# maropu/spark-data-repair-plugin

Measured on AMD Instinct MI355X. Metric: repaired cells/sec, higher is better.
Workload: dtype f32 gradients (LightGBM's score_t), exact int64 fixed-point histogram sums, f64 scores

## Files before the change

### spark-data-repair-plugin_amd/csrc/rgbm.hip

```cpp
#include <hip/hip_runtime.h>
#include <algorithm>
#include <atomic>
#include <condition_variable>
#include <chrono>
#include <cmath>
#include <cstdio>
#include <cstdlib>
#include <cstring>
#include <deque>
#include <map>
#include <memory>
#include <stdexcept>
#include <mutex>
#include <string>
#include <thread>
#include <vector>

#include "rgbm_host.h"
#include "rgbm_kernels.h"
#include "rgbm_level.h"
#include "rgbm_small.h"


namespace {
using rgh::fail; using rgh::DevBuf; using rgh::use_device; using rgh::StreamGuard; using rgh::guarded;
using rgh::AR_I64; using rgh::AR_U32; using rgh::AR_I32; using rgh::all_reduce; using rgh::all_gather_on; using rgh::stream_sync_watchdog; using rgh::comm_abort;
using rgh::comm_kind; using rgh::comm_rank; using rgh::comm_nranks; using rgh::upload_pinned;

struct Feat {
    int32_t n_codes = 0, V = 0, has_nan = 0; std::vector<int32_t> ub;
    std::vector<uint32_t> unseen;
    bool is_unseen(int32_t c) const { return !unseen.empty() && ((unseen[(size_t)c >> 5] >> (c & 31)) & 1u); }
};
struct Tree {
    int32_t L = 1;
    double *gain = nullptr, *leaf_value = nullptr;
    int32_t *feat = nullptr, *theta = nullptr, *dleft = nullptr, *left = nullptr, *right = nullptr, *leaf_count = nullptr;
    std::unique_ptr<double[]> own;
    static size_t doubles(int L) { const size_t n = (size_t)L - 1; return n + (size_t)L + (5 * n + (size_t)L + 1) / 2; }
    void place(double* p, int L_) {
        L = L_; const size_t n = (size_t)L - 1;
        gain = p; leaf_value = p + n;
        int32_t* q = reinterpret_cast<int32_t*>(p + n + L);
        feat = q; theta = q + n; dleft = q + 2 * n; left = q + 3 * n; right = q + 4 * n; leaf_count = q + 5 * n;
    }
    void alloc(int L_) { own.reset(new double[doubles(L_)]); place(own.get(), L_); }
};

struct DeviceModel {
    DevBuf<rg::PNode> nodes; DevBuf<double> leaf_value;
    DevBuf<uint32_t> qs_masks, qs_used; DevBuf<double> qs_leaves; DevBuf<int32_t> qs_foff; int qs_S = 0, qs_MW = 0;
    DevBuf<uint8_t> lut; DevBuf<long long> lut_off; DevBuf<int32_t> n_codes; DevBuf<uint8_t> miss; DevBuf<int32_t> ident;
    int node_stride = 1, leaf_stride = 1;
};

}

struct rgbm_model {
    int32_t objective = 0, num_class = 0, K = 1, n_iter = 0, F = 0;
    std::vector<Feat> feats;
    std::vector<Tree> trees;
    std::unique_ptr<double[]> tree_arena;
    std::mutex mu;
    std::map<int, DeviceModel*> dev;
    ~rgbm_model() { for (auto& kv : dev) { (void)hipSetDevice(kv.first); delete kv.second; } }
};


namespace {

int32_t mid_code(int32_t a, int32_t b, const double* vals) {
    if (!vals) return (int32_t)(((int64_t)a + (int64_t)b) / 2);
    const double m = (vals[a] + vals[b]) / 2.0;
    int32_t lo = a, hi = b - 1;
    while (lo < hi) { const int32_t c = lo + (hi - lo + 1) / 2; if (vals[c] <= m) lo = c; else hi = c - 1; }
    return lo;
}

int greedy_find_bin(const std::vector<int32_t>& dv, const std::vector<int64_t>& cnt, int max_bin, int64_t total_cnt,
                    int min_data_in_bin, std::vector<int32_t>& ub, const double* vals) {
    const int nd = (int)dv.size();
    ub.clear();
    if (nd <= 0) return 0;
    if (nd <= max_bin) {
        int64_t cur = 0;
        for (int i = 0; i + 1 < nd; ++i) {
            cur += cnt[i];
            if (cur >= min_data_in_bin) { ub.push_back(mid_code(dv[i], dv[i + 1], vals)); cur = 0; }
        }
        ub.push_back(INT32_MAX);
        return (int)ub.size();
    }
    if (min_data_in_bin > 0) {
        max_bin = (int)std::min<int64_t>(max_bin, total_cnt / min_data_in_bin);
        max_bin = std::max(max_bin, 1);
    }
    double mean_bin_size = (double)total_cnt / max_bin;
    int rest_bin_cnt = max_bin;
    int64_t rest_sample_cnt = total_cnt;
    std::vector<char> big(nd, 0);
    for (int i = 0; i < nd; ++i)
        if ((double)cnt[i] >= mean_bin_size) { big[i] = 1; --rest_bin_cnt; rest_sample_cnt -= cnt[i]; }
    mean_bin_size = (double)rest_sample_cnt / rest_bin_cnt;
    std::vector<int32_t> upper(max_bin, INT32_MAX), lower(max_bin, INT32_MAX);
    int bin_cnt = 0;
    lower[0] = dv[0];
    int64_t cur = 0;
    for (int i = 0; i + 1 < nd; ++i) {
        if (!big[i]) rest_sample_cnt -= cnt[i];
        cur += cnt[i];
        double half = mean_bin_size * 0.5f;
        if (half < 1.0) half = 1.0;
        if (big[i] || (double)cur >= mean_bin_size || (big[i + 1] && (double)cur >= half)) {
            upper[bin_cnt] = dv[i];
            ++bin_cnt;
            lower[bin_cnt] = dv[i + 1];
            if (bin_cnt >= max_bin - 1) break;
            cur = 0;
            if (!big[i]) { --rest_bin_cnt; mean_bin_size = (double)rest_sample_cnt / (double)rest_bin_cnt; }
        }
    }
    ++bin_cnt;
    for (int i = 0; i + 1 < bin_cnt; ++i) {
        int32_t v = mid_code(upper[i], lower[i + 1], vals);
        if (ub.empty() || ub.back() != v) ub.push_back(v);
    }
    ub.push_back(INT32_MAX);
    return (int)ub.size();
}

void find_bin(const unsigned int* cnt, int32_t n_codes, int64_t n_train, const rgbm_params& p, Feat& f, const double* vals) {
    std::vector<int32_t> dv; std::vector<int64_t> dc;
    int64_t seen = 0;
    for (int32_t c = 0; c < n_codes; ++c) if (cnt[c]) { dv.push_back(c); dc.push_back(cnt[c]); seen += cnt[c]; }
    const int64_t na = n_train - seen;
    int mb = p.max_bin - (na > 0 ? 1 : 0) - 1;
    if (mb < 1) mb = 1;
    f.n_codes = n_codes; f.has_nan = na > 0 ? 1 : 0;
    f.V = greedy_find_bin(dv, dc, mb, seen, p.min_data_in_bin, f.ub, vals);
}


constexpr double DISTINCT_MAX_RATIO = 0.5;
constexpr long long DISTINCT_MIN_ROWS = 1ll << 20;
struct RunSwitches {
    int grower = 0;
    bool timing = false;
    int lv_lds = 0;
    long long lv_blocks = 0;
    long long mt_blocks = 0;
    int mt_T = 0;
    int mt_rep = 8;
    bool joint_root = true;
    bool mt_acc2 = true;
    bool mt_sparse = true;
    int mt_rot = -1;
    int mt_rot_copies2 = 16;
    int mt_rot_tmin = 2;
    bool fx_separate = false;
    bool distinct = true;
    double distinct_max_ratio = DISTINCT_MAX_RATIO;
    long long distinct_min_rows = DISTINCT_MIN_ROWS;
};
RunSwitches read_switches() {
    RunSwitches w;
    if (const char* e = getenv("RGBM_GROWER")) w.grower = strcmp(e, "leafwise") == 0 ? 2 : (strcmp(e, "level") == 0 ? 1 : 0);
    if (const char* e = getenv("RGBM_LV_LDS")) w.lv_lds = atoi(e);
    if (const char* e = getenv("RGBM_LV_BLOCKS")) w.lv_blocks = atoll(e);
    if (const char* e = getenv("RGBM_MT_BLOCKS")) w.mt_blocks = atoll(e);
    if (const char* e = getenv("RGBM_MT_TREES")) w.mt_T = atoi(e);
    if (const char* e = getenv("RGBM_MT_REP")) w.mt_rep = atoi(e);
    if (const char* e = getenv("RGBM_JOINT_ROOT")) w.joint_root = atoi(e) != 0;
    if (const char* e = getenv("RGBM_MT_ACC2")) w.mt_acc2 = atoi(e) != 0;
    if (const char* e = getenv("RGBM_MT_SPARSE")) w.mt_sparse = atoi(e) != 0;
    if (const char* e = getenv("RGBM_FX_MEASURE")) w.fx_separate = strcmp(e, "separate") == 0;
    if (const char* e = getenv("RGBM_MT_ROT")) w.mt_rot = atoi(e);
    if (const char* e = getenv("RGBM_MT_ROT_COPIES2")) w.mt_rot_copies2 = atoi(e);
    if (const char* e = getenv("RGBM_MT_ROT_TMIN")) w.mt_rot_tmin = atoi(e);
    if (const char* e = getenv("RGBM_DISTINCT")) w.distinct = atoi(e) != 0;
    if (const char* e = getenv("RGBM_DISTINCT_MAX_RATIO")) { const double r = atof(e); if (r >= 0.0 && r <= 1.0) w.distinct_max_ratio = r; }
    if (const char* e = getenv("RGBM_DISTINCT_MIN_ROWS")) w.distinct_min_rows = std::max(1ll, atoll(e));
    w.timing = getenv("RGBM_TIMING") != nullptr;
    return w;
}

struct LgbRand {
    uint32_t x;
    explicit LgbRand(uint32_t seed) : x(seed) {}
    int rnd16() { x = 214013u * x + 2531011u; return (int)((x >> 16) & 0x7FFF); }
    int rnd32() { x = 214013u * x + 2531011u; return (int)(x & 0x7FFFFFFF); }
    float next_float() { return (float)rnd16() / 32768.0f; }
    int next_int(int lo, int hi) { return rnd32() % (hi - lo) + lo; }
    std::vector<int> sample(int N, int K) {
        std::vector<int> ret;
        if (K > N || K <= 0) return ret;
        if (K == N) { for (int i = 0; i < N; ++i) ret.push_back(i); return ret; }
        if (K > 1 && (double)K > ((double)N / std::log2((double)K))) {
            for (int i = 0; i < N; ++i) {
                double prob = (double)(K - (int)ret.size()) / (double)(N - i);
                if (next_float() < prob) ret.push_back(i);
            }
            return ret;
        }
        std::vector<char> in(N, 0);
        for (int r = N - K; r < N; ++r) { int v = next_int(0, r); if (in[v]) in[r] = 1; else in[v] = 1; }
        for (int i = 0; i < N; ++i) if (in[i]) ret.push_back(i);
        return ret;
    }
};


void check_params(const rgbm_params& p) {
    if (p.objective < 0 || p.objective > 2) throw std::invalid_argument("objective must be 0 (binary), 1 (multiclass) or 2 (regression)");
    if (p.max_bin < 2 || p.max_bin > 255) throw std::invalid_argument("max_bin must be in [2, 255]");
    if (p.num_leaves < 2 || p.num_leaves > 32767) throw std::invalid_argument("num_leaves must be in [2, 32767]");
    if (p.n_estimators < 1) throw std::invalid_argument("n_estimators must be positive");
    if (!(p.learning_rate > 0.0)) throw std::invalid_argument("learning_rate must be positive");
    if (p.objective == 2 && p.learning_rate > 1.0) throw std::invalid_argument("regression with learning_rate > 1 is not supported");
    if (p.objective == 1 && p.num_class < 2) throw std::invalid_argument("multiclass needs num_class >= 2");
    if (p.min_data_in_leaf < 0 || p.lambda_l1 < 0 || p.lambda_l2 < 0) throw std::invalid_argument("negative regularisation / min_data_in_leaf");
    if (p.bagging_fraction <= 0.0 || p.bagging_fraction > 1.0) throw std::invalid_argument("bagging_fraction must be in (0, 1]");
    if (p.feature_fraction <= 0.0 || p.feature_fraction > 1.0) throw std::invalid_argument("feature_fraction must be in (0, 1]");
}

struct HostLabelStats {
    bool valid = false;
    std::vector<double> tot; double suml = 0.0, w_max = 0.0;
};

struct FitHost {
    int64_t n_train = 0; int nchunk = 1; size_t lds_hist = 0;
    std::vector<int32_t> cols, ncod; std::vector<long long> cnt_off, lut_off; std::vector<unsigned int> cnt;
    std::vector<rg::FeatMeta> fmeta; std::vector<rg::ChunkMeta> cmeta; std::vector<uint8_t> lut, miss, trivial;
    std::vector<double> init, yv32; rg::TrainConst tc;
    std::unique_ptr<rgbm_model> model;
};

void fit_setup(const rgbm_table& tab, const double* y_value_in, const double* class_weight, const HostLabelStats* hls, const rgbm_params& p, int32_t F, FitHost& h) {
    using namespace rg;
    const int64_t N = tab.n;
    const int obj = p.objective;
    const std::vector<int32_t>& cols = h.cols; const std::vector<int32_t>& ncod = h.ncod; const std::vector<long long>& cnt_off = h.cnt_off;
    const std::vector<unsigned int>& cnt = h.cnt;
    const int n_y = ncod[F];
    const int K = obj == 1 ? p.num_class : 1;
    const double* y_value = nullptr;
    if (obj == 2) { h.yv32.resize(std::max(n_y, 1)); for (int c = 0; c < n_y; ++c) h.yv32[c] = (double)(float)y_value_in[c]; y_value = h.yv32.data(); }
    const unsigned int* ycnt = cnt.data() + cnt_off[F];
    int64_t& n_train = h.n_train; n_train = 0;
    for (int c = 0; c < n_y; ++c) n_train += ycnt[c];
    if (n_train <= 0) throw std::out_of_range("no training rows (every target cell is NULL)");
    if (N >= (1ll << 31) - 4096) throw std::invalid_argument("more than 2^31 rows per table are not supported");

    h.model.reset(new rgbm_model());
    rgbm_model* model = h.model.get();
    model->objective = obj; model->num_class = obj == 1 ? K : (obj == 0 ? 2 : 1); model->K = K; model->F = F;
    model->feats.resize(F);
    std::vector<FeatMeta>& fmeta = h.fmeta; fmeta.assign(F, FeatMeta());
    std::vector<long long>& lut_off = h.lut_off; lut_off.assign(F + 1, 0);
    std::vector<uint8_t>& miss = h.miss; std::vector<uint8_t>& trivial = h.trivial; miss.assign(F, 0); trivial.assign(F, 0);
    int totbins = 0;
    for (int f = 0; f < F; ++f) {
        Feat& ft = model->feats[f];
        const std::vector<double>* cv = (size_t)cols[f] < tab.col_values.size() ? &tab.col_values[cols[f]] : nullptr;
        find_bin(cnt.data() + cnt_off[f], ncod[f], n_train, p, ft, (cv && (int32_t)cv->size() == ncod[f] && ncod[f] > 0) ? cv->data() : nullptr);
        if ((size_t)cols[f] < tab.col_kind.size() && tab.col_kind[cols[f]] == 1) {
            const unsigned int* cf = cnt.data() + cnt_off[f];
            bool any = false;
            for (int32_t c = 0; c < ncod[f]; ++c) any |= cf[c] == 0;
            if (any) {
                ft.unseen.assign((size_t)(ncod[f] + 31) / 32, 0u);
                for (int32_t c = 0; c < ncod[f]; ++c) if (cf[c] == 0) ft.unseen[(size_t)c >> 5] |= 1u << (c & 31);
            }
        }
        fmeta[f].V = ft.V; fmeta[f].has_nan = ft.has_nan; fmeta[f].nbins = std::max(ft.V + ft.has_nan, 1); fmeta[f].hoff = totbins;
        totbins += fmeta[f].nbins;
        trivial[f] = (ft.V + ft.has_nan <= 1) || ft.V == 0;
        miss[f] = (uint8_t)(ft.has_nan ? ft.V : 0);
        lut_off[f + 1] = lut_off[f] + std::max(ncod[f], 1);
    }
    std::vector<uint8_t>& lut = h.lut; lut.assign(lut_off[F], 0);
    for (int f = 0; f < F; ++f) {
        const Feat& ft = model->feats[f];
        int b = 0;
        for (int c = 0; c < ncod[f]; ++c) { while (b < ft.V - 1 && c > ft.ub[b]) ++b; lut[lut_off[f] + c] = (uint8_t)(ft.V > 0 ? b : 0); }
    }
    const int nchunk = (F + 15) / 16; h.nchunk = nchunk;
    std::vector<ChunkMeta>& cmeta = h.cmeta; cmeta.assign(nchunk, ChunkMeta());
    size_t& lds_hist = h.lds_hist; lds_hist = 0;
    for (int ch = 0; ch < nchunk; ++ch) {
        ChunkMeta& cm = cmeta[ch]; cm.first_feat = ch * 16; cm.nfeat = std::min(16, F - ch * 16); cm.fast_slots = 0; cm.wide_bins = 0;
        for (int j = 0; j < cm.nfeat; ++j) {
            FeatMeta& m = fmeta[ch * 16 + j];
            int sh = 0; while (sh < 5 && (m.nbins << (sh + 1)) <= 256) ++sh;
            m.rep_shift = sh; m.fast_base = cm.fast_slots; m.wide_off = cm.wide_bins;
            cm.fast_slots += m.nbins << sh; cm.wide_bins += m.nbins;
        }
        lds_hist = std::max(lds_hist, (size_t)cm.fast_slots * 16);
    }

    const int nl = std::max({n_y, obj == 0 ? 2 : 1, obj == 1 ? K : 1});
    std::vector<double> tot(nl, 0.0);
    double w_max = 0.0;
    if (hls && hls->valid) { tot = hls->tot; tot.resize(nl, 0.0); w_max = hls->w_max; }
    else {
        for (int c = 0; c < n_y; ++c) {
            const double cw32 = class_weight ? (double)(float)class_weight[c] : 1.0;
            tot[c] = (double)ycnt[c] * cw32;
            if (ycnt[c]) w_max = std::max(w_max, cw32);
        }
    }
    if (!(w_max > 0.0)) w_max = 1.0;
    double sumw = 0.0;
    for (int c = 0; c < nl; ++c) sumw += tot[c];
    std::vector<double>& init = h.init; init.assign(K, 0.0);
    double ymin = 0.0, ymax = 0.0;
    const double keps = k_eps();
    if (obj == 2) {
        bool first = true; double suml = 0.0;
        for (int c = 0; c < n_y; ++c) {
            if (!ycnt[c]) continue;
            if (first) { ymin = ymax = y_value[c]; first = false; }
            ymin = std::min(ymin, y_value[c]); ymax = std::max(ymax, y_value[c]);
        }
        if (hls && hls->valid) suml = hls->suml; else for (int c = 0; c < nl; ++c) suml += tot[c] * (c < n_y ? y_value[c] : 0.0);
        init[0] = suml / sumw;
    } else if (obj == 0) {
// ... 319 lines not shown
        const int L = h.L[t];
        const int32_t* left = h.left + t * (NL - 1); const int32_t* right = h.right + t * (NL - 1);
        if (root_done) { rows += N; root_rows += N; }
        std::vector<int64_t> fin(h.cnt + t * NL, h.cnt + t * NL + NL);
        std::vector<int64_t> nodecnt(std::max(L - 1, 1), 0);
        auto sub = [&](int ch) -> int64_t { return ch < 0 ? fin[~ch] : nodecnt[ch]; };
        for (int j = L - 2; j >= 0; --j) nodecnt[j] = sub(left[j]) + sub(right[j]);
        std::vector<int> node_depth(std::max(L - 1, 1), 0);
        for (int j = 0; j < L - 1; ++j) {
            const int lc = left[j], rc = right[j];
            if (lc >= 0) node_depth[lc] = node_depth[j] + 1;
            if (rc >= 0) node_depth[rc] = node_depth[j] + 1;
            const int64_t a = sub(lc), b = sub(rc);
            bool go = j + 2 < NL;
            if (p.max_depth > 0 && node_depth[j] + 1 >= p.max_depth) go = false;
            if (a < (int64_t)p.min_data_in_leaf * 2 && b < (int64_t)p.min_data_in_leaf * 2) go = false;
            if (go) rows += std::min(a, b);
        }
    }
    stats->hist_rows = rows; stats->root_rows = root_rows;
    stats->hist_bytes = rows * ((int64_t)F + 8) + (rows - root_rows) * 4;
}

void check_fit_args(const rgbm_table& tab, int32_t target_col, const int32_t* feat_cols, int32_t F, const double* y_value, const rgbm_params& p) {
    check_params(p);
    if (F <= 0) throw std::invalid_argument("no feature columns");
    if (target_col < 0 || target_col >= tab.c) throw std::invalid_argument("target column out of range");
    for (int f = 0; f < F; ++f) if (feat_cols[f] < 0 || feat_cols[f] >= tab.c) throw std::invalid_argument("feature column out of range");
    const int obj = p.objective, n_y = tab.n_codes[target_col];
    if (obj == 1 && n_y > p.num_class) throw std::out_of_range("target has more label codes than num_class");
    if (obj == 0 && n_y > 2) throw std::out_of_range("binary objective with more than 2 label codes");
    if (obj == 2 && !y_value) throw std::out_of_range("regression needs the y_value dictionary");
}

struct BinRecords {
    DevBuf<int32_t> cols, ncod; DevBuf<long long> cnt_off; DevBuf<unsigned int> cnt;
    DevBuf<rg::FeatMeta> fmeta; DevBuf<rg::ChunkMeta> cmeta; DevBuf<long long> lut_off; DevBuf<uint8_t> lut, miss; DevBuf<uint4> rec;
    void count_codes(const rgbm_table& tab, int32_t target_col, const int32_t* feat_cols, int32_t F, FitHost& h, hipStream_t s) {
        h.cols.assign(feat_cols, feat_cols + F); h.cols.push_back(target_col);
        h.ncod.resize(F + 1); h.cnt_off.assign(F + 2, 0);
        for (int f = 0; f <= F; ++f) { h.ncod[f] = tab.n_codes[h.cols[f]]; h.cnt_off[f + 1] = h.cnt_off[f] + std::max(h.ncod[f], 1); }
        cols.alloc(F + 1); ncod.alloc(F + 1); cnt_off.alloc(F + 2); cnt.alloc(h.cnt_off[F + 1]);
        cols.upload(h.cols.data(), F + 1, s); ncod.upload(h.ncod.data(), F + 1, s); cnt_off.upload(h.cnt_off.data(), F + 2, s); cnt.zero(s);
        const int gx = (int)std::min<int64_t>((tab.n + 255) / 256, 1024);
        hipLaunchKernelGGL(rg::k_count_codes, dim3(gx, F + 1), dim3(256), 0, s, tab.codes.p, (long long)tab.n, tab.codes.p + (long long)target_col * tab.n, cols.p, ncod.p,
                           cnt_off.p, cnt.p, tab.has_mult ? tab.mult.p : (const uint8_t*)nullptr);
    }
    void download_counts(FitHost& h, hipStream_t s) const { h.cnt.resize(cnt.n); cnt.download(h.cnt.data(), cnt.n, s); }
    void fill(const FitHost& h, long long N, hipStream_t s) {
        const int F = h.tc.F;
        fmeta.alloc(F); cmeta.alloc(h.nchunk); lut_off.alloc(F + 1); lut.alloc(h.lut.size()); miss.alloc(F);
        fmeta.upload(h.fmeta.data(), F, s); cmeta.upload(h.cmeta.data(), h.nchunk, s); lut_off.upload(h.lut_off.data(), F + 1, s);
        lut.upload(h.lut.data(), h.lut.size(), s); miss.upload(h.miss.data(), F, s);
        rec.alloc((size_t)h.nchunk * N);
    }
    void pack(const rgbm_table& t, const uint8_t* lut_, const uint8_t* miss_, uint4* out, const uint8_t* mult, hipStream_t s) const {
        hipLaunchKernelGGL(rg::k_pack_bins, dim3((unsigned)((t.n + 255) / 256)), dim3(256), 0, s, t.codes.p, (long long)t.n, 0ll, (long long)t.n, cols.p, ncod.p,
                           lut_off.p, lut_, miss_, (int)fmeta.n, (int)cmeta.n, out, mult);
    }
    void pack(const rgbm_table& tab, hipStream_t s) { pack(tab, lut.p, miss.p, rec.p, tab.has_mult ? tab.mult.p : (const uint8_t*)nullptr, s); }
};

struct BagState {
    DevBuf<unsigned int> blk, rand, bagcnt; DevBuf<int32_t> sorted_rows, oob; DevBuf<uint8_t> inbag;
    std::vector<unsigned int> seeds;
    long long off = 0, local = 0, nrb = 1;
    void order_rows(const int32_t* d_ycol, long long N, long long n_train, hipStream_t s) {
        const long long nblk = (N + 1023) / 1024;
        blk.alloc(nblk); sorted_rows.alloc(n_train); oob.alloc(n_train); inbag.alloc(N); bagcnt.alloc(2);
        hipLaunchKernelGGL(rg::k_block_count, dim3((unsigned)nblk), dim3(256), 0, s, d_ycol, N, blk.p);
        hipLaunchKernelGGL(rg::k_block_scan, dim3(1), dim3(1024), 0, s, blk.p, nblk);
        hipLaunchKernelGGL(rg::k_stable_compact, dim3((unsigned)nblk), dim3(256), 0, s, d_ycol, N, blk.p, sorted_rows.p);
    }
    void seed(const rgbm_params& p, long long bag_off, long long bag_local, hipStream_t s) {
        off = bag_off; local = bag_local;
        nrb = std::max<long long>(1, (off + local + 1023) / 1024 - off / 1024);
        LgbRand sr2((uint32_t)p.seed); sr2.rnd16();
        const int bagging_seed = sr2.rnd16();
        seeds.resize(nrb);
        for (long long b = 0; b < nrb; ++b) seeds[b] = (unsigned int)(bagging_seed + off / 1024 + b);
        rand.alloc(nrb); rand.upload(seeds.data(), nrb, s);
    }
};

struct TreeBlock {
    DevBuf<int32_t> L, feat, theta, dleft, left, right, cnt, any; DevBuf<double> gain, val;
    void alloc(size_t NT, int NL, int NE, hipStream_t s) {
        const size_t nn = NT * (size_t)(NL - 1), nl = NT * (size_t)NL;
        any.alloc(NE); any.zero(s);
        L.alloc(NT); feat.alloc(nn); theta.alloc(nn); dleft.alloc(nn); left.alloc(nn); right.alloc(nn); cnt.alloc(nl); gain.alloc(nn); val.alloc(nl);
        cnt.zero(s); val.zero(s);
    }
    rg::TreeOut out() const { return rg::TreeOut{L.p, feat.p, theta.p, dleft.p, left.p, right.p, gain.p, val.p, cnt.p}; }
    void host_layout(size_t (&off)[11]) const {
        const size_t bytes[10] = {L.n * 4, feat.n * 4, theta.n * 4, dleft.n * 4, left.n * 4, right.n * 4, cnt.n * 4, gain.n * 8, val.n * 8, any.n * 4};
        off[0] = 0;
        for (int i = 0; i < 10; ++i) off[i + 1] = off[i] + ((bytes[i] + 63) & ~(size_t)63);
    }
    size_t host_bytes() const { size_t off[11]; host_layout(off); return off[10]; }
    HostTrees download(char* base, hipStream_t s) const {
        size_t off[11]; host_layout(off);
        auto get = [&](const auto& buf, int i) { auto* h = reinterpret_cast<decltype(buf.p)>(base + off[i]); buf.download(h, buf.n, s); return h; };
        return HostTrees{get(L, 0), get(feat, 1), get(theta, 2), get(dleft, 3), get(left, 4), get(right, 5), get(cnt, 6), get(gain, 7), get(val, 8), get(any, 9)};
    }
};

struct FitState {
    const rgbm_table& tab; const rgbm_params& p; hipStream_t s; const int32_t F;
    const RunSwitches sw = read_switches();
    const int K = p.objective == 1 ? p.num_class : 1, NL = p.num_leaves, NE = p.n_estimators; const int64_t N = tab.n;
    const bool use_bagging = p.bagging_freq > 0 && p.bagging_fraction < 1.0;
    const bool level_mode = p.max_depth >= 1 && p.max_depth <= rg::LV_MAX_DEPTH && F <= 255 && sw.grower != 2;
    const bool dp = (p.reserved & RGBM_FLAG_ROW_SHARDED) != 0;
    const int32_t* d_ycol; const uint8_t* d_mult = tab.has_mult ? tab.mult.p : (const uint8_t*)nullptr;
    FitHost h; BinRecords bins;
    DevBuf<int32_t> base;
    DevBuf<unsigned int> counter;
    DevBuf<float2> gh;
    DevBuf<double> score, init;
    DevBuf<unsigned long long> fxq;
    DevBuf<rg::FxScale> fxs;
    DevBuf<unsigned long long> qpart; long long fx_parts = 0; bool fx_fused = false;
    TreeBlock trees;
    DevBuf<double> cw, yv, sw_rows; DevBuf<uint8_t> used;
    BagState bag; DevBuf<unsigned int> bagcnt_g;
    const unsigned int* n_in_ptr = nullptr;
    DevBuf<int32_t> it;
    HistTimers timers;

    FitState(const rgbm_table& tab_, int32_t target_col, int32_t F_, const rgbm_params& p_, bool timed, hipStream_t s_)
        : tab(tab_), p(p_), s(s_), F(F_), d_ycol(tab_.codes.p + (long long)target_col * tab_.n), timers{timed, s_} {}

    int grad_gx() const { return (int)std::min<long long>((N + 255) / 256, 4096); }
    bool mc_tile() const { return p.objective == 1 && K >= 16 && K <= 112; }
    bool mc_rows() const { return p.objective == 1 && K < 16; }
    void alloc_fx_parts() {
        if (sw.fx_separate || (p.objective == 1 && !mc_tile() && !mc_rows())) return;
        fx_fused = true; fx_parts = mc_tile() ? (N + 63) / 64 : (mc_rows() ? ((N + 255) / 256) * 4 : (long long)grad_gx());
        qpart.alloc((size_t)fx_parts * K * 2);
    }
    void enqueue_grad(uint8_t* node0, long long NS);
    void enqueue_bagging();
};

struct LevelGrower {
    FitState& st; hipStream_t s;
    int root_feats;
    unsigned long long statrows = 0;
    rg::LevelConst lc, lcj; LevelPassPlan passes;
    const int n_hnodes = (1 << st.p.max_depth) - 1;
    bool use_reduce = false;
    bool joint_root = false; int vtotbins = 0;
    DevBuf<rg::FeatMeta> vfmeta; DevBuf<rg::ChunkMeta> vcmeta; DevBuf<uint4> rec_j; DevBuf<rg::HistBin> part_j, red_j; DevBuf<rg::JointFeat> jf; DevBuf<int16_t> binfeat;
    DevBuf<uint8_t> node; DevBuf<rg::LvPlan> plan; DevBuf<rg::SNode> snodes; DevBuf<rg::Cand> lcand;
    DevBuf<rg::HistBin> part, lpool, part_red; DevBuf<int32_t> count, count_g, err, leafnode; DevBuf<double> ndelta; DevBuf<unsigned long long> d_statrows;
    const int score_gx = (int)std::max<long long>(1, std::min<long long>((st.N + 1023) / 1024, (2048 + st.K - 1) / st.K));
    LevelTrace trace;
    int32_t h_err = 0;
    std::vector<rg::RootLayout> h_root_lay; std::vector<rg::MtLayout> h_mt_lay; std::vector<int> mt_lay_keys;
    DevBuf<rg::RootLayout> root_lay; DevBuf<rg::MtLayout> mt_lay;
    static int mt_lay_key(const MtLaunch& L) { return L.ch * 4 + (L.acc2 ? 2 : 0) + (L.rot ? 1 : 0); }
    int mt_lay_index(const MtLaunch& L) const {
        for (size_t i = 0; i < mt_lay_keys.size(); ++i) if (mt_lay_keys[i] == mt_lay_key(L)) return (int)i;
        return -1;
    }

    explicit LevelGrower(FitState& st_) : st(st_), s(st_.s), root_feats(st_.F), trace(true, st_.K, st_.s) {
        using namespace rg;
        memset(&lc, 0, sizeof(lc)); memset(&lcj, 0, sizeof(lcj));
        lc.lds_bytes = level_lds_bytes(st.sw);
        lc.nchunk = st.h.nchunk; lc.K = st.K; lc.F = st.F; lc.totbins = st.h.tc.totbins;
        lc.num_leaves = st.NL; lc.max_depth = st.p.max_depth; lc.min_data_in_leaf = st.p.min_data_in_leaf; lc.N = st.N; lc.NS = (st.N + 255) & ~255ll; lc.NG = lc.NS;
        lc.sib_local = (st.dp && comm_rank() == 0) ? 1 : 0;
        lc.has_mult = st.tab.has_mult ? 1u : 0u;
        passes = plan_level_passes(st.sw, st.h.fmeta, st.h.cmeta, st.N, st.K, st.p.max_depth, st.tab.has_mult, lc.lds_bytes);
        lc.gx = passes.root_gx; lc.xcd_blocks = 1; lc.max_built = 1;
        node.alloc((size_t)st.K * lc.NS);
        HIPCHK(hipMemsetAsync(node.p, 0xFF, (size_t)st.K * lc.NS, s));
        plan.alloc(st.K); snodes.alloc((size_t)st.K * 256); lcand.alloc((size_t)st.K * 256 * st.F);
        part.alloc(passes.part_items * st.h.tc.totbins); lpool.alloc((size_t)st.K * n_hnodes * st.h.tc.totbins);
        count.alloc((size_t)st.K * 256); use_reduce = st.dp || lc.gx > 4;
        if (st.dp) count_g.alloc((size_t)st.K * 256);
        const int max_built_all = 1 << std::max(0, st.p.max_depth - 2);
        part_red.alloc((size_t)st.K * max_built_all * st.h.tc.totbins + (size_t)st.K * 128 );
        leafnode.alloc((size_t)st.K * LV_MAX_LEAVES); err.alloc(1); err.zero(s); ndelta.alloc((size_t)st.K * 256); d_statrows.alloc(1); d_statrows.zero(s);
        if (st.sw.joint_root && ((long long)st.K * st.N >= (1ll << 21) || (st.tab.has_mult && st.h.nchunk == 2))) {
            const JointRootPlan jp = plan_joint_root(st.h.fmeta, st.h.tc.totbins, st.tab.has_mult, lc.lds_bytes);
            if (jp.on) {
                const int VF = (int)jp.vfm.size();
                joint_root = true; vtotbins = jp.vcm.wide_bins;
                vfmeta.alloc(VF); vfmeta.upload(jp.vfm.data(), VF, s); vcmeta.alloc(1); vcmeta.upload(&jp.vcm, 1, s);
                jf.alloc(st.F); jf.upload(jp.jf.data(), st.F, s); binfeat.alloc(jp.binfeat.size()); binfeat.upload(jp.binfeat.data(), jp.binfeat.size(), s);
                rec_j.alloc((size_t)st.N);
                hipLaunchKernelGGL(k_pack_joint, dim3((unsigned)((st.N + 255) / 256)), dim3(256), 0, s, st.bins.rec.p, (long long)st.N, st.F, jf.p, rec_j.p, st.tab.has_mult ? st.h.nchunk - 1 : -1);
                part_j.alloc((size_t)st.K * lc.gx * vtotbins); red_j.alloc((size_t)st.K * vtotbins + (size_t)st.K * 128 );
                lcj = lc; lcj.nchunk = 1; lcj.F = VF; lcj.totbins = vtotbins; lcj.max_built = 1;
                h_root_lay.resize(1); root_layout_fill(h_root_lay[0], jp.vfm.data(), VF, lc.lds_bytes);
                use_reduce = true; root_feats = VF;
                HIPCHK(hipStreamSynchronize(s));
            }
        }
        if (st.tab.has_mult && st.h.nchunk == 2 && !joint_root)
            throw std::invalid_argument("a two-chunk table with row multiplicities needs the joint-bin root pass (its record carries the multiplicity); this feature set does not pack into 15 groups");
        if (!joint_root) {
            h_root_lay.resize(st.h.nchunk);
            for (int ch = 0; ch < st.h.nchunk; ++ch) root_layout_fill(h_root_lay[ch], st.h.fmeta.data() + st.h.cmeta[ch].first_feat, st.h.cmeta[ch].nfeat, lc.lds_bytes);
        }
        root_lay.alloc(h_root_lay.size()); root_lay.upload(h_root_lay.data(), h_root_lay.size(), s);
        lc.root_lay = root_lay.p; lcj.root_lay = root_lay.p;
        for (int level = 1; level < st.p.max_depth; ++level) for (const auto& L : passes.mt[level]) if (mt_lay_index(L) < 0) {
            const bool acc2 = L.acc2 != 0;
            const ChunkMeta& cm = st.h.cmeta[L.ch];
            const int nf_last = acc2 ? st.h.cmeta[1].nfeat : cm.nfeat;
            const bool li_in_rec = nf_last <= 15 && !st.tab.has_mult;
            mt_lay_keys.push_back(mt_lay_key(L)); h_mt_lay.emplace_back();
            mt_layout_fill(h_mt_lay.back(), st.h.fmeta.data() + cm.first_feat, cm.nfeat, acc2 ? st.h.fmeta.data() + st.h.cmeta[1].first_feat : nullptr, acc2 ? st.h.cmeta[1].nfeat : 0,
                           cm.wide_bins, L.rot != 0, mt_hist_bytes(lc.lds_bytes, acc2 ? MT_THREADS_ACC2 : LV_THREADS, acc2, acc2, !li_in_rec));
        }
        if (!h_mt_lay.empty()) { mt_lay.alloc(h_mt_lay.size()); mt_lay.upload(h_mt_lay.data(), h_mt_lay.size(), s); }
        if (st.sw.timing) {
            fprintf(stderr, "[rgbm] root: gx %d joint %d groups %d\n", lc.gx, joint_root ? 1 : 0, joint_root ? lcj.F : 0);
            for (int level = 1; level < st.p.max_depth; ++level) for (const auto& L : passes.mt[level])
                fprintf(stderr, "[rgbm] level %d launch: chunk %d slots %d..%d route %d T %d G %d gx %d acc2 %d rot %d\n", level, L.ch, L.slot0, L.slot0 + L.nslots - 1, L.route, L.T, L.G, L.gx, L.acc2, L.rot);
        }
        rgh::once_per_device(st.tab.device, rgh::ONCE_LEVEL_LDS, [] {
            HIPCHK(hipFuncSetAttribute((const void*)rg::k_level_root, hipFuncAttributeMaxDynamicSharedMemorySize, rg::LV_LDS_BYTES));
            for (const MtForm& f : MT_FORMS) for (int bag = 0; bag < 2; ++bag) for (int route = 0; route < 2; ++route)
                HIPCHK(hipFuncSetAttribute((const void*)mt_kernel(f, bag != 0, route != 0), hipFuncAttributeMaxDynamicSharedMemorySize, rg::LV_LDS_BYTES));
        });
        if (trace.on) trace.buf.alloc(((size_t)st.K * n_hnodes * st.h.tc.totbins * 16 + (size_t)st.K * 256 * (sizeof(SNode) + 4) + (size_t)st.K * sizeof(LvPlan) + 4096) * (size_t)(st.p.max_depth + 1) * (size_t)(trace.hi - trace.lo + 1) + (size_t)st.NE * 64 + 4096);
    }

    void trace_level(int level) {
        trace.copy("count", level, count.p, (size_t)st.K * 256 * 4);
        trace.copy("plan", level, plan.p, (size_t)st.K * sizeof(rg::LvPlan));
        trace.copy("snodes", level, snodes.p, (size_t)st.K * 256 * sizeof(rg::SNode));
        trace.copy("lpool", level, lpool.p, (size_t)st.K * n_hnodes * st.h.tc.totbins * 16);
    }
    std::pair<const rg::HistBin*, rg::LevelConst> exchange(bool root, int nb, const rg::LevelConst& lp) {
        using namespace rg;
        if (root && !use_reduce) return {part.p, lp};
        if (root && joint_root) {
            hipLaunchKernelGGL(k_level_reduce, dim3((vtotbins + 63) / 64, 1, st.K), dim3(256), 0, s, part_j.p, red_j.p, plan.p, count.p, 1, 1, lcj);
            hipLaunchKernelGGL(k_level_marginal, dim3((st.h.tc.totbins + 255) / 256, st.K), dim3(256), 0, s, red_j.p, part_red.p, plan.p, count.p, jf.p, binfeat.p, vtotbins, lc);
        } else
            hipLaunchKernelGGL(k_level_reduce, dim3((st.h.tc.totbins + 63) / 64, nb, st.K), dim3(256), 0, s, part.p, part_red.p, plan.p, count.p, root ? 1 : 0, nb, lp);
        if (st.dp) {
            const size_t nh = (size_t)st.K * nb * st.h.tc.totbins * 2;
            all_reduce(part_red.p, nh + (size_t)st.K * 256, AR_I64, s);
            hipLaunchKernelGGL(k_counts_unpack, dim3(st.K), dim3(256), 0, s, reinterpret_cast<const long long*>(part_red.p) + nh, count_g.p);
        }
        LevelConst r = lp; r.gx = 1; r.max_built = nb;
        return {part_red.p, r};
    }
    void enqueue_iteration(int it) {
        using namespace rg;
        const TreeOut to = st.trees.out();
        trace.cur_it = it;
        trace.sum("gh", st.gh.p, (size_t)st.K * st.h.tc.NG * 8);
        hipLaunchKernelGGL(k_level_init, dim3(st.K), dim3(64), 0, s, plan.p, snodes.p, count.p, st.n_in_ptr, (long long)st.h.n_train, st.fxq.p, st.h.tc.fx, st.fxs.p, lc);
        int32_t* cntg = st.dp ? count_g.p : count.p;
        st.timers.timed(true, [&]() {
            if (joint_root)
                hipLaunchKernelGGL(k_level_root, dim3((unsigned)lc.gx * (unsigned)st.K, 1, 1), dim3(LV_THREADS), lc.lds_bytes, s, rec_j.p, st.gh.p, node.p, plan.p, part_j.p,
                                   vfmeta.p, vcmeta.p, st.fxs.p, lcj);
            else
                hipLaunchKernelGGL(k_level_root, dim3((unsigned)lc.gx * (unsigned)st.K, 1, st.h.nchunk), dim3(LV_THREADS), lc.lds_bytes, s, st.bins.rec.p, st.gh.p, node.p, plan.p, part.p,
                                   st.bins.fmeta.p, st.bins.cmeta.p, st.fxs.p, lc);
        });
        {
            auto ex = exchange(true, 1, lc);
            hipLaunchKernelGGL(k_level_split<true>, dim3((st.F + 3) / 4, 1, st.K), dim3(256), 0, s, ex.first, lpool.p, plan.p, snodes.p, cntg, count.p, st.bins.fmeta.p,
                               st.used.p, lcand.p, d_statrows.p, st.it.p, n_hnodes, st.fxs.p, st.h.tc, ex.second);
            trace_level(0);
        }
        for (int level = 1; level < st.p.max_depth; ++level) {
            hipLaunchKernelGGL(k_level_plan, dim3(st.K), dim3(256), 0, s, plan.p, snodes.p, lcand.p, st.bins.fmeta.p, level, st.h.tc, lc);
            LevelConst lp = lc;
            lp.xcd_blocks = 0; lp.gx = passes.mt_gx[level]; lp.max_built = 1 << (level - 1);
            for (const MtLaunch& L : passes.mt[level]) {
                LevelConst l1 = lp;
                l1.mt_T = L.T; l1.mt_G = L.G; l1.mt_ch = L.ch; l1.mt_slot0 = L.slot0; l1.mt_nslots = L.nslots; l1.mt_route = L.route; l1.mt_sparse = st.sw.mt_sparse ? 1 : 0;
                l1.mt_lay = mt_lay.p + mt_lay_index(L);
                const bool acc2 = L.acc2 != 0;
                const MtForm form{acc2 ? 2 : (st.h.nchunk <= 2 ? st.h.nchunk : 0), acc2 ? MT_THREADS_ACC2 : LV_THREADS, acc2, acc2, L.rot != 0};
                st.timers.timed(false, [&]() {
                    launch_level_mt(form, st.use_bagging, L.route != 0, dim3((unsigned)L.G * (unsigned)L.gx), s, st.bins.rec.p, st.gh.p, node.p, st.bag.inbag.p,
                                    plan.p, part.p, count.p, st.bins.fmeta.p, st.bins.cmeta.p, err.p, st.fxs.p, l1);
                });
            }
            auto ex = exchange(false, 1 << (level - 1), lp);
            hipLaunchKernelGGL(k_level_split<false>, dim3((st.F + 1) / 2, 1 << (level - 1), st.K), dim3(256), 0, s, ex.first, lpool.p, plan.p, snodes.p,
                               cntg, count.p, st.bins.fmeta.p, st.used.p, lcand.p, d_statrows.p, st.it.p, n_hnodes, st.fxs.p, st.h.tc, ex.second);
            trace_level(level);
        }
        hipLaunchKernelGGL(k_level_plan, dim3(st.K), dim3(256), 0, s, plan.p, snodes.p, lcand.p, st.bins.fmeta.p, st.p.max_depth, st.h.tc, lc);
        hipLaunchKernelGGL(k_level_replay, dim3(st.K), dim3(64), 0, s, plan.p, snodes.p, cntg, to, st.init.p, ndelta.p, leafnode.p, st.trees.any.p, err.p, st.it.p, st.h.tc);
        hipLaunchKernelGGL(k_level_final, dim3(score_gx, st.K), dim3(256), 0, s, st.bins.rec.p, node.p, st.bag.inbag.p, plan.p, to, ndelta.p, st.score.p, count.p, st.it.p, lc);
        if (st.dp) { hipLaunchKernelGGL(k_copy_i32, dim3(st.K), dim3(256), 0, s, count.p, count_g.p, (long long)st.K * 256); all_reduce(count_g.p, (size_t)st.K * 256, AR_I32, s); }
        hipLaunchKernelGGL(k_level_leafcount, dim3(st.K), dim3(LV_MAX_LEAVES), 0, s, plan.p, cntg, leafnode.p, to, st.it.p, st.h.tc);
        trace_level(st.p.max_depth);
        trace.sum("score", st.score.p, (size_t)st.K * st.N * 8); trace.sum("node", node.p, (size_t)st.K * lc.NS);
        hipLaunchKernelGGL(k_next_iteration, dim3(1), dim3(1), 0, s, st.it.p);
    }
    void enqueue_report() { err.download(&h_err, 1, s); d_statrows.download(&statrows, 1, s); }
    void report(int32_t target_col) {
        trace.write(target_col);
        if (h_err & 2) throw std::runtime_error("level grower: a level pass was launched with more built nodes / route entries than its workgroup tables hold (sizing violated)");
        if (h_err) throw std::runtime_error("level grower: a node outside the speculative expansion was selected (expansion bound violated)");
    }
};

struct LeafwiseGrower {
    FitState& st; hipStream_t s;
    DevBuf<int32_t> idx0, idx1, sorted; DevBuf<rg::HistBin> pool; DevBuf<rg::TreeState> state; DevBuf<rg::Leaf> leaves; DevBuf<rg::Cand> cand; DevBuf<double> upd;
    const long long root_tiles = (st.N + rg::TILE_ROWS - 1) / rg::TILE_ROWS;
    const int hist_gx = (int)std::max<long long>(1, std::min<long long>(root_tiles, (1536 + (long long)st.K * st.h.nchunk - 1) / ((long long)st.K * st.h.nchunk)));
    const int part_gx = (int)std::max<long long>(1, std::min<long long>((st.h.n_train + 1023) / 1024, (1024 + st.K - 1) / st.K));
    const int upd_gx = (int)std::max<long long>(1, std::min<long long>((st.h.n_train + 255) / 256, (2048 + st.K - 1) / st.K));
    const size_t upd_lds = (size_t)(3 * st.NL + (st.NL & 1)) * 4 + (size_t)st.NL * 8;

    explicit LeafwiseGrower(FitState& st_) : st(st_), s(st_.s) {
        idx0.alloc((size_t)st.K * st.h.n_train); idx1.alloc((size_t)st.K * st.h.n_train);
        pool.alloc((size_t)st.K * st.NL * st.h.tc.totbins);
        state.alloc(st.K); leaves.alloc((size_t)st.K * st.NL); cand.alloc((size_t)st.K * 2 * st.F);
        upd.alloc((size_t)st.K * st.NL); sorted.alloc((size_t)st.K * st.NL * 3);
        if (st.h.lds_hist > 64 * 1024)
            rgh::once_per_device(st.tab.device, rgh::ONCE_HIST_LDS, [] { HIPCHK(hipFuncSetAttribute((const void*)rg::k_hist, hipFuncAttributeMaxDynamicSharedMemorySize, 160 * 1024)); });
        if (st.h.lds_hist > 160 * 1024) throw std::invalid_argument("histogram working set exceeds LDS");
    }
    void enqueue_iteration(int it) {
        using namespace rg;
        const TreeOut to = st.trees.out();
        const uint8_t* usedp = st.used.p + (size_t)it * st.K * st.F;
        hipLaunchKernelGGL(k_init_iter, dim3(st.K), dim3(64), 0, s, state.p, leaves.p, pool.p, to, st.n_in_ptr, it, st.h.tc);
        for (int step = 0; step < st.NL - 1; ++step) {
            st.timers.timed(step == 0, [&]() {
                hipLaunchKernelGGL(k_hist, dim3(hist_gx, st.K, st.h.nchunk), dim3(256), st.h.lds_hist, s, st.bins.rec.p, st.gh.p, idx0.p, idx1.p, st.base.p,
                                   state.p, pool.p, st.bins.fmeta.p, st.bins.cmeta.p, st.fxs.p, st.h.tc);
            });
            hipLaunchKernelGGL(k_split_find, dim3((st.F + 3) / 4, st.K), dim3(256), 0, s, pool.p, state.p, leaves.p, st.bins.fmeta.p, usedp, cand.p, st.fxs.p, st.h.tc);
            hipLaunchKernelGGL(k_tree_step, dim3(st.K), dim3(64), 0, s, state.p, leaves.p, cand.p, pool.p, st.bins.fmeta.p, to, it, st.h.tc);
            hipLaunchKernelGGL(k_partition, dim3(part_gx, st.K), dim3(256), 0, s, reinterpret_cast<const uint8_t*>(st.bins.rec.p), idx0.p, idx1.p, st.base.p, state.p, st.h.tc);
            hipLaunchKernelGGL(k_finish_split, dim3(st.K), dim3(64), 0, s, state.p, leaves.p, to, it, st.h.tc);
        }
        hipLaunchKernelGGL(k_finalize_tree, dim3(st.K), dim3(64), 0, s, state.p, leaves.p, to, st.init.p, upd.p, sorted.p, st.trees.any.p, it, st.h.tc);
        hipLaunchKernelGGL(k_score_update, dim3(upd_gx, st.K), dim3(256), upd_lds, s, state.p, leaves.p, sorted.p, upd.p, idx0.p, idx1.p, st.base.p, st.score.p, st.n_in_ptr, st.h.tc);
        if (st.use_bagging)
            hipLaunchKernelGGL(k_score_update_oob, dim3(upd_gx, st.K), dim3(256), 0, s, reinterpret_cast<const uint8_t*>(st.bins.rec.p), st.bag.oob.p, st.bag.bagcnt.p,
                               state.p, to, st.bins.fmeta.p, upd.p, st.score.p, it, st.h.tc);
    }
};

void FitState::enqueue_grad(uint8_t* node0, long long NS) {
    using namespace rg;
    if (p.objective == 0) hipLaunchKernelGGL(k_grad<0>, dim3(grad_gx()), dim3(256), 0, s, score.p, d_ycol, yv.p, cw.p, sw_rows.p, bag.inbag.p, gh.p, node0, NS, qpart.p, d_mult, h.tc);
    else if (mc_rows())
        hipLaunchKernelGGL(k_grad_mc_rows<256>, dim3((unsigned)((N + 255) / 256)), dim3(256), (size_t)K * 256 * 8, s, score.p, d_ycol, cw.p, sw_rows.p, bag.inbag.p, gh.p, node0, NS, qpart.p, d_mult, h.tc);
    else if (mc_tile())
        hipLaunchKernelGGL(k_grad_mc, dim3((unsigned)((N + 63) / 64)), dim3(256), (size_t)(K * 64 + 320) * 8, s, score.p, d_ycol, cw.p, sw_rows.p, bag.inbag.p, gh.p, node0, NS, qpart.p, d_mult, h.tc);
    else if (p.objective == 1) hipLaunchKernelGGL(k_grad<1>, dim3(grad_gx()), dim3(256), 0, s, score.p, d_ycol, yv.p, cw.p, sw_rows.p, bag.inbag.p, gh.p, node0, NS, (unsigned long long*)nullptr, d_mult, h.tc);
    else hipLaunchKernelGGL(k_grad<2>, dim3(grad_gx()), dim3(256), 0, s, score.p, d_ycol, yv.p, cw.p, sw_rows.p, bag.inbag.p, gh.p, node0, NS, qpart.p, d_mult, h.tc);
    if (fx_fused) {
        const long long total = fx_parts * K * 2;
        const unsigned gx = (unsigned)std::max<long long>(1, std::min<long long>(256, (total + 8191) / 8192));
        hipLaunchKernelGGL(k_fx_reduce, dim3(gx), dim3(256), (size_t)K * 2 * 8, s, qpart.p, fx_parts, 2 * K, fxq.p);
    } else {
        const unsigned gx = (unsigned)std::max<long long>(1, std::min<long long>(128, (N + 4095) / 4096));
        hipLaunchKernelGGL(k_fx_measure, dim3(gx, K), dim3(256), 0, s, gh.p, (long long)N, (long long)h.tc.NG, h.tc.fx, fxq.p, d_mult);
    }
    if (dp) all_reduce(fxq.p, (size_t)K * 2, AR_I64, s);
    if (!level_mode) hipLaunchKernelGGL(k_fx_scale, dim3(1), dim3(256), 0, s, fxq.p, K, h.tc.fx, fxs.p);
}
void FitState::enqueue_bagging() {
    using namespace rg;
    hipLaunchKernelGGL(k_bagging, dim3((unsigned)((bag.nrb + 63) / 64)), dim3(64), 0, s, bag.rand.p, bag.local, p.bagging_fraction, bag.sorted_rows.p, bag.inbag.p, bag.bagcnt.p,
                       bag.off, (long long)h.n_train);
    hipLaunchKernelGGL(k_bag_lists, dim3((unsigned)((std::max<long long>(bag.local, 1) + 255) / 256)), dim3(256), 0, s, bag.sorted_rows.p, bag.local, bag.inbag.p, base.p, bag.oob.p, bag.bagcnt.p);
    if (dp) {
        hipLaunchKernelGGL(k_copy_i32, dim3(1), dim3(256), 0, s, reinterpret_cast<const int32_t*>(bag.bagcnt.p), reinterpret_cast<int32_t*>(bagcnt_g.p), 2ll);
        all_reduce(bagcnt_g.p, 2, AR_U32, s);
    }
}

rgbm_model* train_core(const rgbm_table& tab, int32_t target_col, const int32_t* feat_cols, int32_t F,
                       const double* y_value, const double* class_weight, const double* sample_weight_host,
                       const HostLabelStats* hls, const rgbm_params& p, rgbm_train_stats* stats, bool view_stats = false) {
    using namespace rg;
    check_fit_args(tab, target_col, feat_cols, F, y_value, p);
    if (F > 65535) throw std::invalid_argument("more than 65535 feature columns");
    StreamGuard sg_; hipStream_t s = sg_.s;
    rgh::Event ev_begin, ev_end;
    HIPCHK(hipEventRecord(ev_begin.e, s));

    FitState st(tab, target_col, F, p, stats != nullptr, s);
    auto now = []() { return std::chrono::duration<double, std::milli>(std::chrono::steady_clock::now().time_since_epoch()).count(); };
    const double t_start = now();
    st.bins.count_codes(tab, target_col, feat_cols, F, st.h, s);
    if (st.dp) {
        if (comm_kind() == 0) throw std::invalid_argument("row-sharded training requested but this thread has no communicator (rgbm_comm_init)");
        all_reduce(st.bins.cnt.p, st.bins.cnt.n, AR_U32, s);
    }
    st.bins.download_counts(st.h, s);
    if (st.dp) stream_sync_watchdog(s); else HIPCHK(hipStreamSynchronize(s));
    fit_setup(tab, y_value, class_weight, hls, p, F, st.h);
    if (p.objective == 2) y_value = st.h.yv32.data();
    const int n_y = st.h.ncod[F];

    const double t_bins = now();
    st.bins.fill(st.h, st.N, s);
    if (tab.has_mult && (!st.level_mode || st.h.nchunk > 2 || (F % 16) == 0 || sample_weight_host || st.use_bagging))
        throw std::invalid_argument("a table with row multiplicities trains with the level grower (1 <= max_depth <= 7), at most 32 features of which the last 16-feature "
                                    "chunk holds at most 15, without bagging and without per-row weights");
    st.bins.pack(tab, s);
    if (st.dp && (!st.level_mode || sample_weight_host))
        throw std::invalid_argument("row-sharded training supports the level grower (1 <= max_depth <= 7) without per-row weights");
    st.counter.alloc(1); st.counter.zero(s);
    if (!st.level_mode || st.use_bagging) {
        st.base.alloc(st.h.n_train);
        hipLaunchKernelGGL(k_iota_train, dim3((unsigned)((st.N + 255) / 256)), dim3(256), 0, s, st.d_ycol, (long long)st.N, st.base.p, st.counter.p);
    }
    if (st.level_mode) st.h.tc.NG = (st.N + 255) & ~255ll;
    st.gh.alloc((size_t)st.K * st.h.tc.NG); st.gh.zero(s);
    st.score.alloc((size_t)st.K * st.N); st.init.alloc(st.K);
    st.init.upload(st.h.init.data(), st.K, s);
    st.fxq.alloc((size_t)st.K * 2); st.fxq.zero(s);
    st.fxs.alloc(st.K);
    hipLaunchKernelGGL(k_init_score, dim3((unsigned)((st.N + 255) / 256)), dim3(256), 0, s, st.score.p, (long long)st.N, st.K, st.init.p);
    const size_t NT = (size_t)st.NE * st.K;
    st.trees.alloc(NT, st.NL, st.NE, s);
    std::unique_ptr<LevelGrower> lg; std::unique_ptr<LeafwiseGrower> lw;
    if (st.level_mode) lg.reset(new LevelGrower(st)); else lw.reset(new LeafwiseGrower(st));
    if (class_weight) { st.cw.alloc(n_y); st.cw.upload(class_weight, n_y, s); }
    if (y_value) { st.yv.alloc(n_y); st.yv.upload(y_value, n_y, s); }
    if (sample_weight_host) { st.sw_rows.alloc(st.N); st.sw_rows.upload(sample_weight_host, st.N, s); }

    const std::vector<uint8_t> used = make_used_masks(p, NT, F, st.h.trivial);
    st.used.alloc(used.size()); st.used.upload(used.data(), used.size(), s);

    if (st.use_bagging) {
        st.bag.order_rows(st.d_ycol, st.N, st.h.n_train, s);
        long long bag_off = 0, bag_local = st.h.n_train;
        if (st.dp) {
            unsigned int h_local = 0; st.counter.download(&h_local, 1, s); stream_sync_watchdog(s);
            bag_local = (long long)h_local;
            std::vector<long long> rc((size_t)comm_nranks(), 0); rc[(size_t)comm_rank()] = bag_local;
            DevBuf<long long> d_rc(rc.size()); d_rc.upload(rc.data(), rc.size(), s);
            all_reduce(d_rc.p, rc.size(), AR_I64, s);
            d_rc.download(rc.data(), rc.size(), s); stream_sync_watchdog(s);
            long long tot = 0;
            for (int r = 0; r < comm_nranks(); ++r) { if (r < comm_rank()) bag_off += rc[(size_t)r]; tot += rc[(size_t)r]; }
            if (tot != st.h.n_train) throw std::runtime_error("row-sharded bagging: the ranks' training-row counts do not add up");
            st.bagcnt_g.alloc(2);
        }
        st.bag.seed(p, bag_off, bag_local, s);
        HIPCHK(hipStreamSynchronize(s));
        st.n_in_ptr = st.dp ? st.bagcnt_g.p : st.bag.bagcnt.p;
    }
    st.it.alloc(1); st.it.zero(s);
    st.alloc_fx_parts();
    unsigned int view_train_rows = 0;
    if (view_stats && stats) {
        hipLaunchKernelGGL(k_count_train, dim3((unsigned)((st.N + 255) / 256)), dim3(256), 0, s, st.d_ycol, (long long)st.N, st.counter.p);
        st.counter.download(&view_train_rows, 1, s);
    }

    if (st.sw.timing) HIPCHK(hipStreamSynchronize(s));
    const double t_setup = now();
    for (int it = 0; it < st.NE; ++it) {
        if (st.use_bagging && it % p.bagging_freq == 0) st.enqueue_bagging();
        st.enqueue_grad(lg ? lg->node.p : nullptr, lg ? lg->lc.NS : 0);
        if (lg) lg->enqueue_iteration(it); else lw->enqueue_iteration(it);
    }
    HIPCHK(hipGetLastError());

    const double t_enq = now();
    std::vector<char> host_trees(st.trees.host_bytes());
    const HostTrees ht = st.trees.download(host_trees.data(), s);
    if (lg) lg->enqueue_report();
    HIPCHK(hipEventRecord(ev_end.e, s));
    if (st.dp) stream_sync_watchdog(s); else HIPCHK(hipStreamSynchronize(s));
    if (st.sw.timing) fprintf(stderr, "[rgbm] target %d K=%d: count+bins %.1f ms, alloc+pack %.1f ms, enqueue %.1f ms, drain+download %.1f ms\n", target_col, st.K, t_bins - t_start, t_setup - t_bins, t_enq - t_setup, now() - t_enq);
    if (lg) lg->report(target_col);

    model_from_trees(st.h.model.get(), ht, st.NE, st.K, st.NL);
    if (stats) {
        float ms = 0.f; HIPCHK(hipEventElapsedTime(&ms, ev_begin.e, ev_end.e));
        const int nranks = st.dp ? comm_nranks() : 1;
        fill_train_stats(stats, ms, st.timers, ht, p, st.level_mode, st.use_bagging, nranks, st.N, st.h.n_train, F, lg ? lg->root_feats : F, st.K, lg ? lg->statrows : 0);
        if (view_stats && st.level_mode && st.h.n_train > 0) {
            const int64_t root_w = stats->root_rows, level_w = std::max<int64_t>(0, stats->hist_rows - root_w);
            stats->root_rows = root_w > 0 ? (int64_t)st.NE * st.K * (int64_t)view_train_rows : 0;
            stats->hist_rows = stats->root_rows + (int64_t)((double)level_w * (double)view_train_rows / (double)st.h.n_train + 0.5);
            stats->hist_bytes = stats->hist_rows * ((int64_t)F + 8);
        }
    }
    return st.h.model.release();
}


struct PredictScratch;
void predict_device(rgbm_model* m, int device, hipStream_t s, const int32_t* d_codes, long long Ntab, long long row0, long long n,
                    const int32_t* d_feat_cols, double* d_proba, int32_t* d_label, double* d_top, PredictScratch* scratch);

struct SmallFitDev {
    FitHost h; int F = 0, K = 1, NL = 0, NE = 0; bool bag = false;
    BinRecords bins; BagState bagst; TreeBlock trees;
    DevBuf<unsigned int> counter; DevBuf<uint8_t> used;
    DevBuf<float2> gh; DevBuf<double> score, init, upd, cw, yv;
    DevBuf<int32_t> idx0, idx1, base, tree_L; DevBuf<rg::HistBin> pool;
    DevBuf<rg::ScanLane> scan_map; std::vector<rg::ScanLane> h_scan; int scan_waves = 0;
    DevBuf<uint4> vrec; DevBuf<double> vscore, vtop; DevBuf<int32_t> vlabel; DevBuf<uint8_t> vlut, vmiss; std::vector<uint8_t> h_vlut, h_vmiss; long long n_valid = 0;
    std::vector<char> host_trees;
    std::vector<uint8_t> h_used;
};

void score_valid_with_model(const rgbm_fit_spec& sp, rgbm_model* m) {
    if (!sp.valid_table || !m || sp.valid_table->n <= 0 || (!sp.valid_label_out && !sp.valid_value_out)) return;
    const rgbm_table& vt = *sp.valid_table;
    StreamGuard sg_; hipStream_t s = sg_.s;
    DevBuf<int32_t> d_fc(sp.n_features), d_lab(vt.n); DevBuf<double> d_top(vt.n);
    d_fc.upload(sp.feat_cols, sp.n_features, s);
    predict_device(m, vt.device, s, vt.codes.p, vt.n, 0, vt.n, d_fc.p, nullptr, d_lab.p, d_top.p, nullptr);
    if (sp.valid_label_out) d_lab.download(sp.valid_label_out, vt.n, s);
    if (sp.valid_value_out) d_top.download(sp.valid_value_out, vt.n, s);
    HIPCHK(hipStreamSynchronize(s));
}

bool small_fit_eligible(const rgbm_table& tab, int32_t F, const rgbm_params& p, long long small_rows) {
    if (tab.n > small_rows || tab.n >= (1ll << 31) - 4096) return false;
    if (tab.has_mult) return false;
    if (p.num_leaves > rg::SM_MAX_LEAVES || F > rg::SM_MAX_FEATS) return false;
    if (p.reserved & RGBM_FLAG_ROW_SHARDED) return false;
    return true;
}

struct HarvestArena {
    std::mutex mu; void* p = nullptr; size_t cap = 0; int device = -1;
    static constexpr size_t KEEP_MAX = (size_t)1 << 30;
    void* get(size_t bytes, int dev) {
        if (bytes == 0 || bytes > KEEP_MAX || getenv("RGBM_NO_PIN") != nullptr) return nullptr;
        if (p && cap >= bytes && device == dev) return p;
        if (p) { (void)hipHostFree(p); p = nullptr; cap = 0; }
        const size_t want = std::min(KEEP_MAX, bytes + bytes / 4);
        if (hipHostMalloc(&p, want, hipHostMallocDefault) != hipSuccess) { (void)hipGetLastError(); p = nullptr; return nullptr; }
        cap = want; device = dev;
        return p;
    }
};
HarvestArena& harvest_arena() { static HarvestArena* a = new HarvestArena(); return *a; }

void train_batch_small(const rgbm_fit_spec* specs, int32_t n_fits, rgbm_model** out, int32_t* status) {
    using namespace rg;
    long long small_rows = 65536;
    if (const char* e = getenv("RGBM_SMALL_ROWS")) small_rows = atoll(e);
    const int device = specs[0].table->device;
    std::vector<int> batch;
    auto record_error = [&](int i, const std::exception& e) { status[i] = rgh::status_of(e); rgh::last_error() = e.what(); };
    auto run_single = [&](int i) {
        const rgbm_fit_spec& sp = specs[i];
        try {
            out[i] = train_core(*sp.table, sp.target_col, sp.feat_cols, sp.n_features, sp.y_value, sp.class_weight, nullptr, nullptr, *sp.params, nullptr); status[i] = RGBM_OK;
            score_valid_with_model(sp, out[i]);
        }
        catch (const std::exception& e) { record_error(i, e); }
    };
    for (int i = 0; i < n_fits; ++i) {
        out[i] = nullptr; status[i] = RGBM_OK;
        const rgbm_fit_spec& sp = specs[i];
        if (!sp.table || !sp.feat_cols || !sp.params) { status[i] = RGBM_ERR_ARG; rgh::last_error() = "rgbm_table_train_batch: bad fit spec"; continue; }
        if (sp.table->device != device) throw std::invalid_argument("rgbm_table_train_batch: all tables of a batch must live on one device");
        if (small_fit_eligible(*sp.table, sp.n_features, *sp.params, small_rows)) batch.push_back(i); else run_single(i);
    }
    if (batch.empty()) return;
    if (batch.size() == 1 && !getenv("RGBM_SMALL_ALWAYS")) { run_single(batch[0]); return; }

    StreamGuard sg_; hipStream_t s = sg_.s;
    const bool timing = getenv("RGBM_TIMING") != nullptr;
    auto now = []() { return std::chrono::duration<double, std::milli>(std::chrono::steady_clock::now().time_since_epoch()).count(); };
    const double t_start = now();
    std::vector<std::unique_ptr<SmallFitDev>> dev(n_fits);
    std::vector<int> live;
    for (int i : batch) {
        const rgbm_fit_spec& sp = specs[i]; const rgbm_table& tab = *sp.table; const rgbm_params& p = *sp.params; const int F = sp.n_features;
        try { check_fit_args(tab, sp.target_col, sp.feat_cols, F, sp.y_value, p); }
        catch (const std::exception& e) { record_error(i, e); continue; }
        dev[i].reset(new SmallFitDev());
        SmallFitDev& d = *dev[i];
        d.F = F; d.K = p.objective == 1 ? p.num_class : 1; d.NL = p.num_leaves; d.NE = p.n_estimators;
        d.bins.count_codes(tab, sp.target_col, sp.feat_cols, F, d.h, s); d.bins.download_counts(d.h, s);
        live.push_back(i);
    }
    HIPCHK(hipStreamSynchronize(s));
    std::vector<int> ok;
    int NE_max = 0; size_t lds_max = 0; long long N_max = 1, ntrain_max = 1, nrb_max = 1, nvalid_max = 0; bool any_bag = false;
    for (int i : live) {
        const rgbm_fit_spec& sp = specs[i]; const rgbm_table& tab = *sp.table; const rgbm_params& p = *sp.params;
        SmallFitDev& d = *dev[i]; FitHost& h = d.h; const int F = d.F, K = d.K, NL = d.NL, NE = d.NE; const long long N = tab.n;
        try {
        fit_setup(tab, sp.y_value, sp.class_weight, nullptr, p, F, h);
        {
            std::vector<ScanLane> sm; int lanes_used = 0;
            for (int f = 0; f < F; ++f) {
                const int nl_f = std::max(1, (h.fmeta[f].V + 3) / 4);
                if (lanes_used % 64 + nl_f > 64) while (lanes_used % 64) { sm.push_back(ScanLane{-1, 0, 1, 0}); ++lanes_used; }
                const int first = lanes_used % 64;
                for (int q = 0; q < nl_f; ++q) { sm.push_back(ScanLane{f, 4 * q, q == 0 ? 1 : 0, first + nl_f - 1}); ++lanes_used; }
            }
            while (lanes_used % 64) { sm.push_back(ScanLane{-1, 0, 1, 0}); ++lanes_used; }
            const int Wn = lanes_used / 64;
            const bool off_switch = getenv("RGBM_SMALL_PACKED") && atoi(getenv("RGBM_SMALL_PACKED")) == 0;
            if (!off_switch && 2 * Wn <= SM_WAVES && h.tc.totbins <= 2048 && sm_lds_bytes(h.lds_hist, NL, F, h.tc.totbins) <= 150 * 1024) { d.scan_waves = Wn; d.h_scan = std::move(sm); }
        }
        const size_t lds = sm_lds_bytes(h.lds_hist, NL, F, d.scan_waves > 0 ? h.tc.totbins : 0);
        if (lds > 160 * 1024 - 2048) { dev[i].reset(); run_single(i); continue; }
        const int nchunk = h.nchunk; const long long n_train = h.n_train;
        d.bins.fill(h, N, s);
        d.bins.pack(tab, s);
        const int32_t* d_ycol = tab.codes.p + (long long)sp.target_col * N;
        d.bag = p.bagging_freq > 0 && p.bagging_fraction < 1.0;
        d.counter.alloc(1); d.counter.zero(s);
        d.base.alloc(n_train);
        hipLaunchKernelGGL(k_iota_train, dim3((unsigned)((N + 255) / 256)), dim3(256), 0, s, d_ycol, N, d.base.p, d.counter.p);
        d.gh.alloc((size_t)K * N); d.gh.zero(s);
        d.score.alloc((size_t)K * N); d.init.alloc(K); d.init.upload(h.init.data(), K, s);
        hipLaunchKernelGGL(k_init_score, dim3((unsigned)((N + 255) / 256)), dim3(256), 0, s, d.score.p, N, K, d.init.p);
        d.idx0.alloc((size_t)K * n_train); d.idx1.alloc((size_t)K * n_train);
        d.pool.alloc((size_t)K * NL * h.tc.totbins); d.upd.alloc((size_t)K * NL); d.tree_L.alloc(K);
        const size_t NT = (size_t)NE * K;
        d.trees.alloc(NT, NL, NE, s);
        const int n_y = h.ncod[F];
        if (sp.class_weight) { d.cw.alloc(n_y); d.cw.upload(sp.class_weight, n_y, s); }
        if (p.objective == 2) { d.yv.alloc(n_y); d.yv.upload(h.yv32.data(), n_y, s); }
        if (d.scan_waves > 0) { d.scan_map.alloc(d.h_scan.size()); d.scan_map.upload(d.h_scan.data(), d.h_scan.size(), s); }
        if (sp.valid_table && sp.valid_table->n > 0 && (sp.valid_label_out || sp.valid_value_out)) {
            const rgbm_table& vt = *sp.valid_table;
            if (vt.c != tab.c) throw std::invalid_argument("rgbm_table_train_batch: valid_table must have the columns of the training table");
            d.n_valid = vt.n;
            d.h_vlut.assign(std::max<size_t>(h.lut.size(), 1), 0); d.h_vmiss.assign(F, 255);
            for (int f = 0; f < F; ++f) {
                const Feat& ft = h.model->feats[f]; int b = 0;
                for (int cde = 0; cde < h.ncod[f]; ++cde) { while (b < ft.V - 1 && cde > ft.ub[b]) ++b; d.h_vlut[h.lut_off[f] + cde] = ft.is_unseen(cde) ? (uint8_t)255 : (uint8_t)(ft.V > 0 ? b : 0); }
            }
            d.vlut.alloc(d.h_vlut.size()); d.vlut.upload(d.h_vlut.data(), d.h_vlut.size(), s); d.vmiss.alloc(F); d.vmiss.upload(d.h_vmiss.data(), F, s);
            d.vrec.alloc((size_t)nchunk * vt.n);
            d.bins.pack(vt, d.vlut.p, d.vmiss.p, d.vrec.p, nullptr, s);
            d.vscore.alloc((size_t)K * vt.n); d.vlabel.alloc(vt.n); d.vtop.alloc(vt.n);
            hipLaunchKernelGGL(k_init_score, dim3((unsigned)((vt.n + 255) / 256)), dim3(256), 0, s, d.vscore.p, (long long)vt.n, K, d.init.p);
            nvalid_max = std::max<long long>(nvalid_max, vt.n);
        }
        d.h_used = make_used_masks(p, NT, F, h.trivial);
        d.used.alloc(d.h_used.size()); d.used.upload(d.h_used.data(), d.h_used.size(), s);
        if (d.bag) {
            d.bagst.order_rows(d_ycol, N, n_train, s);
            d.bagst.seed(p, 0, n_train, s);
            any_bag = true; nrb_max = std::max(nrb_max, d.bagst.nrb);
        }
        NE_max = std::max(NE_max, NE); lds_max = std::max(lds_max, lds); N_max = std::max(N_max, N); ntrain_max = std::max(ntrain_max, n_train);
        ok.push_back(i);
        }
        catch (const std::exception& e) { (void)hipStreamSynchronize(s); record_error(i, e); dev[i].reset(); continue; }
    }
    if (ok.empty()) return;
    if (timing) HIPCHK(hipStreamSynchronize(s));
    const double t_setup = now();
    std::vector<SmallFit> fits(ok.size()); std::vector<int32_t> tree2fit;
    for (size_t j = 0; j < ok.size(); ++j) {
        const int i = ok[j]; const rgbm_fit_spec& sp = specs[i]; const rgbm_params& p = *sp.params; SmallFitDev& d = *dev[i]; FitHost& h = d.h;
        SmallFit& f = fits[j]; memset(&f, 0, sizeof(f));
        f.c = h.tc; f.rec = d.bins.rec.p; f.ycol = sp.table->codes.p + (long long)sp.target_col * sp.table->n; f.gh = d.gh.p; f.score = d.score.p;
        f.idx0 = d.idx0.p; f.idx1 = d.idx1.p; f.base_idx = d.base.p; f.pool = d.pool.p; f.fmeta = d.bins.fmeta.p; f.cmeta = d.bins.cmeta.p; f.used = d.used.p;
        f.out = d.trees.out();
        f.init = d.init.p; f.upd = d.upd.p; f.tree_L = d.tree_L.p; f.any_split = d.trees.any.p;
        f.class_w = sp.class_weight ? d.cw.p : nullptr; f.y_value = p.objective == 2 ? d.yv.p : nullptr;
        f.rand_state = d.bagst.rand.p; f.sorted_rows = d.bagst.sorted_rows.p; f.inbag = d.bagst.inbag.p; f.bagcnt = d.bagst.bagcnt.p; f.oob = d.bagst.oob.p;
        f.bag_fraction = p.bagging_fraction; f.bag_nrb = d.bagst.nrb; f.bag_freq = d.bag ? p.bagging_freq : 0;
        f.tree0 = (int32_t)tree2fit.size(); f.n_estimators = d.NE; f.lds_hist = (unsigned long long)h.lds_hist;
        f.scan_map = d.scan_map.p; f.scan_waves = d.scan_waves;
        f.vrec = d.vrec.p; f.vscore = d.vscore.p; f.n_valid = d.n_valid;
        for (int k = 0; k < d.K; ++k) tree2fit.push_back((int32_t)j);
    }
    DevBuf<unsigned long long> d_prof(8); d_prof.zero(s);
    for (auto& f : fits) f.prof = d_prof.p;
    DevBuf<SmallFit> d_fits(fits.size()); DevBuf<int32_t> d_t2f(tree2fit.size());
    d_fits.upload(fits.data(), fits.size(), s); d_t2f.upload(tree2fit.data(), tree2fit.size(), s);
    rgh::once_per_device(device, rgh::ONCE_SMALL_TREE_LDS, [] { HIPCHK(hipFuncSetAttribute((const void*)k_small_tree, hipFuncAttributeMaxDynamicSharedMemorySize, 160 * 1024 - 2048)); });
    if (lds_max > 160 * 1024 - 2048) throw std::invalid_argument("small-table batch: histogram working set exceeds LDS");
    const unsigned nf = (unsigned)fits.size(), KT = (unsigned)tree2fit.size();
    const unsigned gx_rows = (unsigned)std::min<long long>((N_max + 255) / 256, 64), gx_train = (unsigned)std::min<long long>((ntrain_max + 255) / 256, 64);
    for (int it = 0; it < NE_max; ++it) {
        if (any_bag) {
            hipLaunchKernelGGL(k_small_bagging, dim3((unsigned)((nrb_max + 63) / 64), nf), dim3(64), 0, s, d_fits.p, it);
            hipLaunchKernelGGL(k_small_bag_lists, dim3(gx_train, nf), dim3(256), 0, s, d_fits.p, it);
        }
        hipLaunchKernelGGL(k_small_grad, dim3(gx_rows, nf), dim3(256), 0, s, d_fits.p, it);
        hipLaunchKernelGGL(k_small_tree, dim3(KT), dim3(SM_THREADS), lds_max, s, d_fits.p, d_t2f.p, it);
        if (any_bag) hipLaunchKernelGGL(k_small_oob, dim3(gx_train, KT), dim3(256), 0, s, d_fits.p, d_t2f.p, it);
        if (nvalid_max > 0) hipLaunchKernelGGL(k_small_valid, dim3((unsigned)std::min<long long>((nvalid_max + 255) / 256, 64), KT), dim3(256), 0, s, d_fits.p, d_t2f.p, it);
    }
    for (int i : ok) {
        SmallFitDev& d = *dev[i]; const rgbm_fit_spec& sp = specs[i];
        if (d.n_valid <= 0) continue;
        hipLaunchKernelGGL(k_softmax_argmax, dim3((unsigned)((d.n_valid + 255) / 256)), dim3(256), 0, s, d.vscore.p, d.n_valid, sp.params->objective,
                           d.h.model->num_class, (double*)nullptr, d.vlabel.p, d.vtop.p);
        if (sp.valid_label_out) d.vlabel.download(sp.valid_label_out, d.n_valid, s);
        if (sp.valid_value_out) d.vtop.download(sp.valid_value_out, d.n_valid, s);
    }
    HIPCHK(hipGetLastError());
    const double t_enq = now();
    if (timing) HIPCHK(hipStreamSynchronize(s));
    const double t_iter = now();
    std::vector<int> want;
    for (int i : ok) if (!((specs[i].params->reserved & RGBM_FLAG_NO_MODEL) && dev[i]->n_valid > 0)) want.push_back(i);
    std::vector<HostTrees> hts(n_fits);
    HarvestArena& HA = harvest_arena();
    std::unique_lock<std::mutex> ha_lock(HA.mu, std::try_to_lock);
    size_t need = 0;
    for (int i : want) need += dev[i]->trees.host_bytes();
    char* base = ha_lock.owns_lock() ? (char*)HA.get(need, device) : nullptr;
    for (int i : want) {
        SmallFitDev& d = *dev[i];
        const size_t bytes = d.trees.host_bytes();
        if (base) { hts[i] = d.trees.download(base, s); base += bytes; }
        else { d.host_trees.resize(bytes); hts[i] = d.trees.download(d.host_trees.data(), s); }
    }
    HIPCHK(hipStreamSynchronize(s));
    const double t_down = now();
    {
        struct Item { int fit; size_t t0, t1; };
        std::vector<Item> items;
        for (int i : want) {
            SmallFitDev& d = *dev[i];
            const size_t n = model_trees_begin(d.h.model.get(), hts[i], d.NE, d.K);
            for (size_t t0 = 0; t0 < n; t0 += 512) items.push_back(Item{i, t0, std::min(n, t0 + 512)});
        }
        std::atomic<size_t> next{0};
        auto work = [&]() {
            for (size_t j = next.fetch_add(1); j < items.size(); j = next.fetch_add(1))
                model_trees_fill(dev[items[j].fit]->h.model.get(), hts[items[j].fit], dev[items[j].fit]->NL, items[j].t0, items[j].t1);
        };
        const size_t nth = std::min<size_t>(std::min<size_t>(std::max<size_t>(items.size(), 1), 32), std::max(1u, std::thread::hardware_concurrency()));
        std::vector<std::thread> th;
        for (size_t q = 1; q < nth; ++q) th.emplace_back(work);
        work();
        for (auto& t : th) t.join();
    }
    for (int i : ok) status[i] = RGBM_OK;
    for (int i : want) out[i] = dev[i]->h.model.release();
#if defined(SM_PROF)
    { unsigned long long hp[8]; d_prof.download(hp, 8, s); HIPCHK(hipStreamSynchronize(s)); unsigned long long tot = 0; for (int q = 0; q < 8; ++q) tot += hp[q];
      fprintf(stderr, "[rgbm] k_small_tree phases (%% of thread-0 cycles): zero %.1f | accumulate %.1f | flush %.1f | split_find %.1f | reduce+pick %.1f | partition %.1f | finish %.1f | score %.1f\n",
              100.0 * hp[0] / tot, 100.0 * hp[1] / tot, 100.0 * hp[2] / tot, 100.0 * hp[3] / tot, 100.0 * hp[4] / tot, 100.0 * hp[5] / tot, 100.0 * hp[6] / tot, 100.0 * hp[7] / tot); }
#endif
    if (timing) fprintf(stderr, "[rgbm] batch of %zu fits, %u class trees, %d iterations: setup %.1f ms, enqueue %.1f ms, iterations drained after %.1f ms, download %.1f ms (%s), models %.1f ms\n",
                        ok.size(), KT, NE_max, t_setup - t_start, t_enq - t_setup, t_iter - t_setup, t_down - t_iter, ha_lock.owns_lock() ? "page-locked block" : "pageable", now() - t_down);
}

template <class Fn> void parallel_ranges(size_t n, size_t min_per_thread, Fn fn) {
    const size_t nth = std::min<size_t>(std::min<size_t>(8, std::max<size_t>(1, n / std::max<size_t>(min_per_thread, 1))), std::max(1u, std::thread::hardware_concurrency()));
    if (nth <= 1) { fn((size_t)0, n); return; }
    std::exception_ptr err; std::mutex emu; std::vector<std::thread> th;
    for (size_t q = 0; q < nth; ++q)
        th.emplace_back([&, q]() { try { fn(n * q / nth, n * (q + 1) / nth); } catch (...) { std::lock_guard<std::mutex> lk(emu); if (!err) err = std::current_exception(); } });
// ... 753 lines not shown
```

### spark-data-repair-plugin_amd/csrc/rgbm_level.h

```cpp
#pragma once
#include "rgbm_kernels.h"

namespace rg {

constexpr int LV_INACTIVE = 255;
constexpr int LV_MAX_EXP = 64;
constexpr int LV_MAX_BUILT = 32;
constexpr int LV_CNT_REP = 16;
constexpr int LV_THREADS = 1024;
constexpr int LV_TILE = 2 * LV_THREADS;
constexpr int LV_LDS_TOTAL = 160 * 1024;
constexpr int LV_LDS_BYTES = LV_LDS_TOTAL;
constexpr int LV_MAX_DEPTH = 7;
constexpr int LV_MAX_LEAVES = 128;

constexpr int MT_MAX_T = 64;
constexpr int MT_MAX_NODES = 128;
constexpr int MT_RT_BUDGET = 256;
constexpr int MT_MAX_RT = MT_RT_BUDGET + MT_MAX_T;
constexpr int MT_WT_ROWS = 256;
constexpr int MT_RING_PLAIN = 128;
constexpr int MT_RING_SPEC = 128;
__host__ __device__ constexpr int mt_ring(bool spec) { return spec ? MT_RING_SPEC : MT_RING_PLAIN; }
constexpr int MT_CNT_REP = 4;

constexpr int MT_THREADS_ACC2 = 768;
#ifndef MT_CONSUMERS_N
#define MT_CONSUMERS_N 4
#endif
constexpr int MT_CONSUMERS = MT_CONSUMERS_N;

struct SNode {
    long long Gq, Hq;
    double pmin;
    int32_t count, depth, parent, is_left;
    int32_t left, right;
    int32_t best_feature, searched;
    int32_t hslot, pad;
    Cand best;
};

struct LvPlan {
    int32_t n_nodes, lvl_first, lvl_end, n_exp, n_built, live_rows , pad1, pad2, pad3, done, error, child_first, n_hslots, pad4;
    long long n_in;
    uint8_t exp[LV_MAX_EXP];
    uint8_t built_is_left[LV_MAX_EXP];
    uint32_t route0[256];
    uint32_t route1[256];
};

struct MtLayout;
struct RootLayout;
struct LevelConst {
    const MtLayout* mt_lay;
    const RootLayout* root_lay;
    int32_t gx;
    int32_t max_built;
    int32_t nchunk, K, F, totbins, num_leaves, max_depth, min_data_in_leaf, lds_bytes;
    int32_t sib_local;
    int32_t xcd_blocks;
    int32_t mt_T, mt_G, mt_ch, mt_slot0, mt_nslots, mt_route;
    int32_t mt_sparse;
    uint32_t has_mult;
    long long N, NS, NG;
};

__device__ __forceinline__ uint32_t rec_byte(const uint4& r, int j) {
    uint32_t w = (j < 8) ? ((j < 4) ? r.x : r.y) : ((j < 12) ? r.z : r.w);
    return (w >> (8 * (j & 3))) & 0xFFu;
}

constexpr int LV_MAX_Q = 11;
__host__ __device__ inline int lv_shift(int nbins, int q) {
    int l = 0; while ((1 << l) < nbins) ++l;
    int s = q - l;
    return s < 0 ? 0 : (s > 5 ? 5 : s);
}

__host__ __device__ inline int lv_slots(const FeatMeta* fm, int nfeat, int q) {
    int t = 0;
    for (int j = 0; j < nfeat; ++j) t += fm[j].nbins << lv_shift(fm[j].nbins, q);
    return t;
}

__host__ __device__ constexpr int mt_rot_dummy(bool rot) { return rot ? 4 : 0; }
__host__ __device__ inline int mt_shift(int nbins, int q, bool rot) { return rot ? (q < 0 ? 0 : (q > 2 ? 2 : q)) : lv_shift(nbins, q); }
__host__ __device__ inline int mt_slots(const FeatMeta* fm, int nfeat, int q, bool rot) {
    int t = 0;
    for (int j = 0; j < nfeat; ++j) t += fm[j].nbins << mt_shift(fm[j].nbins, q, rot);
    return t;
}
__host__ __device__ constexpr int mt_max_q(bool rot) { return rot ? 2 : LV_MAX_Q; }

constexpr int LV_ROOT_FIXED = 256;
#if !defined(MT_SPARSE_DIV_N)
#define MT_SPARSE_DIV_N 16
#endif
constexpr long long MT_SPARSE_DIV = MT_SPARSE_DIV_N;
__host__ __device__ constexpr long long mt_fixed_bytes(int threads, bool acc2, bool spec = false, bool li = true ) {
    return ((!acc2 && !spec) ? (long long)MT_MAX_T * 8  : 0) + (long long)MT_MAX_T * 32 + MT_MAX_NODES + 16 + 512 + 256 + (long long)(MT_MAX_T + 2) * 8 + (long long)MT_MAX_RT * 8 + (long long)MT_MAX_NODES * MT_CNT_REP * 4 + (long long)MT_MAX_NODES * 8 +
           (long long)(threads / 64 - (spec ? MT_CONSUMERS : 0)) * mt_ring(spec) * ((acc2 ? 32 : 16) + 8 + (li ? 2 : 0)) + 256;
}
__host__ __device__ constexpr long long mt_hd(int threads, bool acc2, bool spec) { return ((LV_LDS_TOTAL - mt_fixed_bytes(threads, acc2, spec, false)) / 2) & ~15ll; }
__host__ __device__ constexpr long long mt_hist_bytes(long long lds_bytes, int threads, bool acc2, bool spec, bool li) {
    const long long fixed = mt_fixed_bytes(threads, acc2, spec, li), hd = mt_hd(threads, acc2, spec);
    const long long room_h = (long long)LV_LDS_TOTAL - fixed - hd;
    const long long x = hd < room_h ? hd : room_h;
    const long long a = lds_bytes - fixed;
    return a < 2 * x ? a : 2 * x;
}

constexpr int MT_LAY_Q = LV_MAX_Q + 1;
struct MtLayout {
    uint32_t q_spn[MT_MAX_NODES + 4];
    int32_t wide[32], hdelta[32];
    int32_t fb[MT_LAY_Q][32];
    int32_t sh[MT_LAY_Q][32];
    uint8_t bin_feat[32 * 256];
};
struct RootLayout { int32_t q, spn, pad0, pad1; int32_t sh[16], fbase[16]; };

inline void mt_layout_fill(MtLayout& L, const FeatMeta* fm, int nfeat, const FeatMeta* fm1 , int nfeat1, int wide_bins0,
                           bool rot, long long avail ) {
    memset(&L, 0, sizeof(L));
    const bool acc2 = fm1 != nullptr;
    auto spn_of = [&](int q) { return mt_slots(fm, nfeat, q, rot) + (acc2 ? mt_slots(fm1, nfeat1, q, rot) : 0) + mt_rot_dummy(rot); };
    for (int tot = 0; tot < MT_MAX_NODES + 4; ++tot) {
        int q = mt_max_q(rot);
        while (q > 0 && (long long)tot * spn_of(q) * 16 > avail) --q;
        L.q_spn[tot] = (uint32_t)q | (uint32_t)spn_of(q) << 8;
    }
    for (int q = 0; q < MT_LAY_Q; ++q) {
        int o = 0;
        for (int a = 0; a < (acc2 ? 2 : 1); ++a) {
            const FeatMeta* fa = a == 0 ? fm : fm1;
            const int na = a == 0 ? nfeat : nfeat1;
            for (int j = 0; j < 16; ++j) {
                int shj = 0, fbj = 0;
                if (j < na) { shj = mt_shift(fa[j].nbins, q, rot); fbj = o; o += fa[j].nbins << shj; }
                L.fb[q][a * 16 + j] = fbj; L.sh[q][a * 16 + j] = shj;
            }
        }
    }
    for (int q = 0; q < 32; ++q) L.wide[q] = 0x7FFFFFFF;
    for (int a = 0; a < (acc2 ? 2 : 1); ++a) {
        const FeatMeta* fa = a == 0 ? fm : fm1;
        const int na = a == 0 ? nfeat : nfeat1;
        for (int j = 0; j < na && j < 16; ++j) {
            const int wide = (a == 0 ? 0 : wide_bins0) + fa[j].wide_off;
            L.wide[a * 16 + j] = wide; L.hdelta[a * 16 + j] = fa[j].hoff - wide;
            for (int b = 0; b < fa[j].nbins && wide + b < 32 * 256; ++b) L.bin_feat[wide + b] = (uint8_t)(a * 16 + j);
        }
    }
}
inline void root_layout_fill(RootLayout& L, const FeatMeta* fm, int nfeat, int lds_bytes) {
    memset(&L, 0, sizeof(L));
    int q = LV_MAX_Q;
    while (q > 0 && (long long)lv_slots(fm, nfeat, q) * 16 + LV_ROOT_FIXED > lds_bytes) --q;
    L.q = q;
    for (int j = 0; j < 16 && j < nfeat; ++j) { L.sh[j] = lv_shift(fm[j].nbins, q); L.fbase[j] = L.spn; L.spn += fm[j].nbins << L.sh[j]; }
}

__global__ __launch_bounds__(64) void k_level_init(LvPlan* __restrict__ plan, SNode* __restrict__ nodes, int32_t* __restrict__ count,
                                                   const unsigned int* __restrict__ n_in_ptr, long long n_train,
                                                   unsigned long long* __restrict__ Q, FxGrid fx, FxScale* __restrict__ fxs, LevelConst c) {
    const int k = blockIdx.x, lane = lane_id();
    if (lane == 0) {
        const int e_g = fx_tree_exponent(Q[2 * k], fx.q_mult, fx.c_g, fx.e_g_min, fx.e_g_max);
        const int e_h = fx_tree_exponent(Q[2 * k + 1], fx.q_mult, fx.c_h, fx.e_h_min, fx.e_h_max);
        FxScale f; f.sg = fx_pow2(e_g); f.sh = fx_pow2(e_h); f.inv_sg = fx_pow2(-e_g); f.inv_sh = fx_pow2(-e_h);
        fxs[k] = f;
        Q[2 * k] = 0ull; Q[2 * k + 1] = 0ull;
    }
    LvPlan* pp = &plan[k];
    const long long n_in = n_in_ptr ? (long long)n_in_ptr[0] : n_train;
    for (int i = lane; i < 256; i += 64) { pp->route0[i] = 0; pp->route1[i] = 0xFFFFFFFFu; count[(long long)k * 256 + i] = 0; }
    if (lane == 0) {
        pp->n_nodes = 1; pp->lvl_first = 0; pp->lvl_end = 1; pp->n_exp = 0; pp->n_built = 1;
        pp->error = 0; pp->child_first = 1; pp->n_hslots = 1; pp->n_in = n_in;
        pp->done = (n_in < (long long)c.min_data_in_leaf * 2) ? 1 : 0;
        SNode r; memset(&r, 0, sizeof(r));
        r.count = (int)n_in; r.depth = 0; r.parent = -1; r.left = -1; r.right = -1; r.best_feature = -1; r.searched = 0; r.hslot = 0;
        r.best.gain = -INFINITY; r.pmin = -INFINITY;
        nodes[(long long)k * 256] = r;
    }
}

__global__ __launch_bounds__(LV_THREADS, 1) void k_level_root(const uint4* __restrict__ rec, const float2* __restrict__ gh, const uint8_t* __restrict__ node,
                                                              const LvPlan* __restrict__ plan, HistBin* __restrict__ part,
                                                              const FeatMeta* __restrict__ fmeta, const ChunkMeta* __restrict__ cmeta,
                                                              const FxScale* __restrict__ fxs , LevelConst c) {
    extern __shared__ __attribute__((aligned(16))) unsigned char smem[];
    int k, bx, nbx;
    if (c.xcd_blocks) { const unsigned id = blockIdx.x, r = id >> 3; k = (int)(r % (unsigned)c.K); bx = (int)(r / (unsigned)c.K) * 8 + (int)(id & 7u); nbx = c.gx; }
    else { k = blockIdx.y; bx = blockIdx.x; nbx = gridDim.x; }
    const int ch = blockIdx.z;
    if (plan[k].done) return;
    const double sg_k = fxs[k].sg, sh_k = fxs[k].sh;
    const ChunkMeta cm = cmeta[ch];
    const FeatMeta* fm = fmeta + cm.first_feat;
    const int tid = threadIdx.x, lane = tid & 63, nfeat = cm.nfeat;
    const RootLayout* lay = c.root_lay + ch;
    int sh[16], fbase[16];
    const int spn = lay->spn;
#pragma unroll
    for (int j = 0; j < 16; ++j) { sh[j] = lay->sh[j]; fbase[j] = lay->fbase[j]; }
    unsigned long long* hist_g = reinterpret_cast<unsigned long long*>(smem);
    unsigned long long* hist_h = hist_g + spn;
    for (int i = tid; i < spn; i += LV_THREADS) reinterpret_cast<uint4*>(smem)[i] = make_uint4(0u, 0u, 0u, 0u);
    int cj[16], sh3[16];
#pragma unroll
    for (int j = 0; j < 16; ++j) { sh3[j] = sh[j] + 3; cj[j] = (fbase[j] + (lane & ((1 << sh[j]) - 1))) * 8; }
    const int hdelta = spn;
    __syncthreads();

    const long long N = c.N;
    const uint8_t* node_in = node + (long long)k * c.NS;
    const uint4* recc = rec + (long long)ch * N;
    const float2* ghk = gh + (long long)k * c.NG;
    const long long ntiles_all = (N + LV_TILE - 1) / LV_TILE;
    const long long tbeg = c.xcd_blocks ? ntiles_all * bx / nbx : bx;
    const long long ntiles = c.xcd_blocks ? ntiles_all * (bx + 1) / nbx : ntiles_all;
    const long long tstep = c.xcd_blocks ? 1 : nbx;

    constexpr int RPT = LV_TILE / LV_THREADS;
    int cur_n[RPT], nxt_n[RPT]; uint4 cur_r[RPT], nxt_r[RPT]; float2 cur_g[RPT], nxt_g[RPT];
    auto fetch = [&](long long t, int (&fn)[RPT], uint4 (&fr)[RPT], float2 (&fg)[RPT]) __attribute__((always_inline)) {
        const bool tv = t < ntiles;
        const long long pb = tv ? t * LV_TILE : 0;
        const long long left_rows = N - pb;
        const unsigned lim = (unsigned)(left_rows < LV_TILE ? left_rows : LV_TILE) - 1u;
#pragma unroll
        for (int q = 0; q < RPT; ++q) {
            const unsigned o = (unsigned)(q * LV_THREADS + tid);
            const unsigned oc = o < lim ? o : lim;
            typedef float v2f __attribute__((ext_vector_type(2)));
            const int nv = (int)__builtin_nontemporal_load(node_in + pb + oc);
            fr[q] = (recc + pb)[oc];
            const v2f gv = __builtin_nontemporal_load(reinterpret_cast<const v2f*>(ghk + pb + oc));
            fg[q] = make_float2(gv.x, gv.y);
            fn[q] = (tv && o <= lim) ? nv : LV_INACTIVE;
        }
    };
    auto accumulate = [&](bool on, const uint4& r, const float2& g) __attribute__((always_inline)) {
        if (on && (g.x != 0.0f || g.y != 0.0f)) {
            unsigned long long gq = (unsigned long long)fx_from_f32(g.x, sg_k), hq = (unsigned long long)fx_from_f32(g.y, sh_k);
            if (c.has_mult) { const unsigned long long m = r.w >> 24; gq *= m; hq *= m; }
            unsigned char* hb = reinterpret_cast<unsigned char*>(hist_g);
            const uint32_t w[4] = {r.x, r.y, r.z, r.w};
#define LV_ATOM(j) { const uint32_t code_ = (w[(j) >> 2] >> (8 * ((j) & 3))) & 0xFFu; \
                     unsigned long long* p_ = reinterpret_cast<unsigned long long*>(hb + cj[j] + (int)(code_ << sh3[j])); \
                     atomicAdd(p_, gq); atomicAdd(p_ + hdelta, hq); }
#pragma unroll
            for (int j = 0; j < 16; ++j) if (j < nfeat) LV_ATOM(j);
#undef LV_ATOM
        }
    };
    long long t = tbeg;
    fetch(t, cur_n, cur_r, cur_g);
    while (t < ntiles) {
        fetch(t + tstep, nxt_n, nxt_r, nxt_g);
#pragma unroll
        for (int q = 0; q < RPT; ++q) accumulate(cur_n[q] != LV_INACTIVE, cur_r[q], cur_g[q]);
        t += tstep; if (t >= ntiles) break;
        fetch(t + tstep, cur_n, cur_r, cur_g);
#pragma unroll
        for (int q = 0; q < RPT; ++q) accumulate(nxt_n[q] != LV_INACTIVE, nxt_r[q], nxt_g[q]);
        t += tstep;
    }
    __syncthreads();
    HistBin* dst = part + (((long long)k * c.gx + bx) * c.max_built) * c.totbins;
    for (int j = 0; j < nfeat; ++j) {
        const int shj = lay->sh[j], fb = lay->fbase[j];
        for (int b = tid; b < fm[j].nbins; b += LV_THREADS) {
            long long tg = 0, th = 0;
            const unsigned long long* sg_ = hist_g + fb + (b << shj); const unsigned long long* sh_ = hist_h + fb + (b << shj);
            for (int r2 = 0; r2 < (1 << shj); ++r2) { tg += (long long)sg_[r2]; th += (long long)sh_[r2]; }
            HistBin o; o.g = tg; o.h = th;
            dst[fm[j].hoff + b] = o;
        }
    }
}

struct MtTree { int32_t base, nlev, rt_off, slot0, nb, live, child_first, k; };

template <int NCHR , bool BAG,
          bool ROUTE ,
          int THREADS , bool ACC2 ,
          bool SPEC ,
          bool ROTP = false >
__global__ __launch_bounds__(THREADS, 1) void k_level_mt(const uint4* __restrict__ rec, const float2* __restrict__ gh, uint8_t* __restrict__ node ,
                                                         const uint8_t* __restrict__ inbag, const LvPlan* __restrict__ plan, HistBin* __restrict__ part,
                                                         int32_t* __restrict__ count, const FeatMeta* __restrict__ fmeta, const ChunkMeta* __restrict__ cmeta,
                                                         int32_t* __restrict__ err_flag,
                                                         const FxScale* __restrict__ fxs , LevelConst c) {
    static_assert(!ACC2 || NCHR == 2, "a two-chunk pass keeps both records in registers");
    static_assert(ACC2 == SPEC && THREADS == (ACC2 ? MT_THREADS_ACC2 : LV_THREADS) && (!ROTP || NCHR == 1 || ACC2) && (NCHR == 0 || NCHR == 1 || NCHR == 2),
                  "k_level_mt: not one of the six launch forms");
    constexpr int WAVES = THREADS / 64;
    constexpr int NCONS = SPEC ? MT_CONSUMERS : 0, NPROD = WAVES - NCONS;
    constexpr int NACC = ACC2 ? 2 : 1;
    constexpr int NRINGS = SPEC ? NPROD : WAVES;
    constexpr int MT_RING = mt_ring(SPEC);
    constexpr bool ROT = ROTP;
    constexpr bool SPARSE = (NCHR == 1) && !ACC2 && !SPEC;
    extern __shared__ __attribute__((aligned(16))) unsigned char smem[];
    const unsigned id = blockIdx.x;
    const int xl = (int)(id & 7u), bslot = (int)(id >> 3);
    const int grp = bslot % c.mt_G, rb = (bslot / c.mt_G) * 8 + xl;
    const int k0 = grp * c.mt_T;
    const int nk = (c.K - k0) < c.mt_T ? (c.K - k0) : c.mt_T;
    const int tid = threadIdx.x, lane = tid & 63, wave = tid >> 6;
    const int ch = ACC2 ? 0 : c.mt_ch;
    constexpr bool route = ROUTE;
    const ChunkMeta cm = cmeta[ch];
    const ChunkMeta cm1 = cmeta[ACC2 ? 1 : ch];
    const int nfeat = cm.nfeat, nfeat1 = ACC2 ? cm1.nfeat : 0;
    const int wb = cm.wide_bins + (ACC2 ? cm1.wide_bins : 0);
    const bool li_in_rec = (ACC2 ? nfeat1 : nfeat) <= 15 && !c.has_mult;
// ... 464 lines not shown
                    const long long row0 = on ? (long long)g * 4 : row_lo;
                    uint4 ra[4], r1[4]; uint32_t bagmask = BAG ? 0u : 0xFu;
#pragma unroll
                    for (int j = 0; j < 4; ++j) {
                        long long rr = row0 + j; if (rr >= N) rr = N - 1;
                        ra[j] = rec_acc[rr]; r1[j] = make_uint4(0, 0, 0, 0);
                        if (BAG) bagmask |= (inbag[rr] ? 1u : 0u) << j;
                    }
                    const uint32_t n4 = on ? *reinterpret_cast<const uint32_t*>(nd_k + row0) : 0xFFFFFFFFu;
                    const float4 g0 = *reinterpret_cast<const float4*>(gh_k + row0), g1 = *reinterpret_cast<const float4*>(gh_k + row0 + 2);
                    uint2 e[4];
                    lookup(n4, tq, e);
                    stage_c(row0, ra, r1, bagmask, n4, g0, g1, e, tq);
                    sp_cnt = 0;
                };
                auto load16 = [&](long long st) __attribute__((always_inline)) -> uint4 {
                    const long long r16 = row_lo + st * 1024 + lane * 16;
                    uint4 v = make_uint4(0xFFFFFFFFu, 0xFFFFFFFFu, 0xFFFFFFFFu, 0xFFFFFFFFu);
                    if (st < nst && r16 < row_hi) v = *reinterpret_cast<const uint4*>(nd_k + r16);
                    return v;
                };
                uint4 n16 = load16(wave);
                for (long long st = wave; st < nst; st += WAVES) {
                    const long long r16 = row_lo + st * 1024 + lane * 16;
                    const uint4 nxt = load16(st + WAVES);
                    const long long left = row_hi - r16;
                    const int nvalid = left >= 16 ? 16 : (left > 0 ? (int)left : 0);
                    const uint32_t w4[4] = {n16.x, n16.y, n16.z, n16.w};
#pragma unroll
                    for (int d = 0; d < 4; ++d) {
                        bool hit = false;
#pragma unroll
                        for (int j = 0; j < 4; ++j) {
                            const uint32_t idx = ((w4[d] >> (8 * j)) & 0xFFu) - base;
                            hit = hit || (idx < nlev && ((xm >> (idx & 63u)) & 1ull) != 0ull && d * 4 + j < nvalid);
                        }
                        const unsigned long long m = __ballot(hit);
                        if (m != 0ull) {
                            const int np = (int)__popcll(m), r_hit = (int)__popcll(m & lane_lt);
                            const int dest = hit ? sp_cnt + r_hit : sp_cnt + np + (lane - r_hit);
                            const uint32_t rx = (uint32_t)__builtin_amdgcn_ds_permute((dest & 63) << 2, (int)(uint32_t)((r16 + d * 4) >> 2));
                            const int rel = (lane - sp_cnt) & 63;
                            if (sp_cnt + np < 64) { if (rel < np) pend = rx; sp_cnt += np; }
                            else {
                                const int rem = sp_cnt + np - 64;
                                if (rel < 64 - sp_cnt) pend = rx;
                                sparse_batch(64);
                                if (lane < rem) pend = rx;
                                sp_cnt = rem;
                            }
                        }
                    }
                    n16 = nxt;
                }
                if (sp_cnt > 0) sparse_batch(sp_cnt);
            }
        }
    }
    if (SPEC) { if (wave < NPROD) { asm volatile("" ::: "memory"); if (lane == 0) { RS_STORE(wave, p_tail); asm volatile("" ::: "memory"); RS_STORE(32 + wave, 1u); } } }
#undef RS_LOAD
#undef RS_STORE
    else while (r_cnt > 0) run_batch(r_cnt < 64 ? r_cnt : 64);
    __syncthreads();
    const uint8_t* __restrict__ bin_feat = reinterpret_cast<const uint8_t*>((uintptr_t)((unsigned long long)(uint32_t)__builtin_amdgcn_readfirstlane((int)rsync[48]) |
                                                                                      (unsigned long long)(uint32_t)__builtin_amdgcn_readfirstlane((int)rsync[49]) << 32));
    for (int i = tid; i < total * wb; i += THREADS) {
        const int ln = i / wb, b = i - ln * wb;
        const MtTree t = ti[nd_tree[ln]];
        const int j = bin_feat[b];
        const int shb = ftab[64 + j], s0 = ftab[32 + j] + ((b - ftab[j]) << shb);
        long long tg = 0, th = 0;
        const unsigned long long* sg_ = hist_g + (size_t)ln * spn + s0; const unsigned long long* sh_ = hist_h + (size_t)ln * spn + s0;
        for (int r2 = 0; r2 < (1 << shb); ++r2) { tg += (long long)sg_[r2]; th += (long long)sh_[r2]; }
        HistBin o; o.g = tg; o.h = th;
        part[(((long long)t.k * c.gx + rb) * c.max_built + (c.mt_slot0 + ln - t.slot0)) * c.totbins + ftab[96 + j] + b] = o;
    }
    if (ch == 0) {
        for (int ln = tid; ln < total; ln += THREADS) {
            int tot = 0;
            for (int r2 = 0; r2 < MT_CNT_REP; ++r2) tot += cnt[ln * MT_CNT_REP + r2];
            const MtTree t = ti[nd_tree[ln]];
            const int ei = c.mt_slot0 + ln - t.slot0;
            if (tot) atomicAdd(&count[(long long)t.k * 256 + t.child_first + 2 * ei + (plan[t.k].built_is_left[ei] ? 0 : 1)], tot);
        }
    }
}

__global__ __launch_bounds__(256) void k_level_reduce(const HistBin* __restrict__ part, HistBin* __restrict__ red, const LvPlan* __restrict__ plan,
                                                      const int32_t* __restrict__ count, int is_root, int nb, LevelConst c) {
    __shared__ long long sg[4][64], sh[4][64];
    const int k = blockIdx.z, bslot = blockIdx.y, bl = threadIdx.x & 63, xl = threadIdx.x >> 6;
    const int b = blockIdx.x * 64 + bl;
    if (blockIdx.x == 0 && blockIdx.y == 0)
        reinterpret_cast<long long*>(red + (long long)c.K * nb * c.totbins)[(long long)k * 256 + threadIdx.x] = (long long)count[(long long)k * 256 + threadIdx.x];
    const LvPlan* pp = &plan[k];
    const int n_built = pp->done ? 0 : (is_root ? 1 : pp->n_built);
    long long ag = 0, ah = 0;
    if (b < c.totbins && bslot < n_built) {
        const HistBin* src = part + (((long long)k * c.gx) * c.max_built + bslot) * c.totbins + b;
        const long long xs = (long long)c.max_built * c.totbins;
#pragma unroll 8
        for (int x = xl; x < c.gx; x += 4) { const HistBin v = src[x * xs]; ag += v.g; ah += v.h; }
    }
    sg[xl][bl] = ag; sh[xl][bl] = ah;
    __syncthreads();
    if (xl == 0 && b < c.totbins) {
        HistBin acc; acc.g = sg[0][bl] + sg[1][bl] + sg[2][bl] + sg[3][bl]; acc.h = sh[0][bl] + sh[1][bl] + sh[2][bl] + sh[3][bl];
        red[((long long)k * nb + bslot) * c.totbins + b] = acc;
    }
}

struct JointFeat { int32_t voff , stride, nbins , nbv , hoff, vbyte , pad0, pad1; };

__global__ __launch_bounds__(256) void k_pack_joint(const uint4* __restrict__ rec, long long N, int F, const JointFeat* __restrict__ jf, uint4* __restrict__ rec_joint,
                                                    int mult_chunk = -1 ) {
    const long long i = (long long)blockIdx.x * 256 + threadIdx.x;
    if (i >= N) return;
    const uint8_t* rec8 = reinterpret_cast<const uint8_t*>(rec);
    uint32_t w[4] = {0, 0, 0, 0};
    for (int f = 0; f < F; ++f) {
        const uint32_t bin = rec8[((long long)(f >> 4) * N + i) * 16 + (f & 15)];
        const int vb = jf[f].vbyte;
        w[vb >> 2] += (bin * (uint32_t)jf[f].stride) << (8 * (vb & 3));
    }
    if (mult_chunk >= 0) w[3] = (w[3] & 0x00FFFFFFu) | ((uint32_t)rec8[((long long)mult_chunk * N + i) * 16 + 15] << 24);
    rec_joint[i] = make_uint4(w[0], w[1], w[2], w[3]);
}

__global__ __launch_bounds__(256) void k_level_marginal(const HistBin* __restrict__ red_j , HistBin* __restrict__ red, const LvPlan* __restrict__ plan,
                                                        const int32_t* __restrict__ count, const JointFeat* __restrict__ jf, const int16_t* __restrict__ bin_feat ,
                                                        int vtotbins, LevelConst c) {
    const int k = blockIdx.y;
    if (blockIdx.x == 0)
        reinterpret_cast<long long*>(red + (long long)c.K * c.totbins)[(long long)k * 256 + threadIdx.x] = (long long)count[(long long)k * 256 + threadIdx.x];
    const int b = blockIdx.x * 256 + threadIdx.x;
    if (b >= c.totbins) return;
    HistBin acc; acc.g = 0; acc.h = 0;
    if (!plan[k].done) {
        const JointFeat f = jf[bin_feat[b]];
        const int digit = b - f.hoff;
        const int period = f.stride * f.nbins;
        const HistBin* src = red_j + (long long)k * vtotbins + f.voff;
        for (int base = digit * f.stride; base < f.nbv; base += period)
            for (int lo = 0; lo < f.stride; ++lo) { const HistBin v = src[base + lo]; acc.g += v.g; acc.h += v.h; }
    }
    red[(long long)k * c.totbins + b] = acc;
}

__global__ __launch_bounds__(256) void k_counts_unpack(const long long* __restrict__ cnt64, int32_t* __restrict__ count_g) {
    const long long i = (long long)blockIdx.x * 256 + threadIdx.x;
    count_g[i] = (int32_t)cnt64[i];
}

template <bool ROOT>
__global__ __launch_bounds__(256) void k_level_split(const HistBin* __restrict__ part, HistBin* __restrict__ pool, LvPlan* __restrict__ plan,
                                                     SNode* __restrict__ nodes, int32_t* __restrict__ count, int32_t* __restrict__ count_local,
                                                     const FeatMeta* __restrict__ fmeta, const uint8_t* __restrict__ used_all ,
                                                     Cand* __restrict__ cand , unsigned long long* __restrict__ stat_rows,
                                                     const int32_t* __restrict__ itp ,
                                                     int n_hnodes, const FxScale* __restrict__ fxs, TrainConst c_model, LevelConst lc) {
    const int k = blockIdx.z, pi = blockIdx.y;
    const TrainConst c = tree_const(c_model, fxs, k);
    const uint8_t* used = used_all + (long long)(*itp) * c.K * c.F;
    const int wv = threadIdx.x >> 6;
    const int f = ROOT ? blockIdx.x * 4 + wv : blockIdx.x * 2 + (wv >> 1);
    const int side = wv & 1;
    const LvPlan* pp = &plan[k];
    if (pp->done) return;
    if (!ROOT && pi >= pp->n_exp) return;
    if (f >= c.F) return;
    const int lane = lane_id();
    const FeatMeta fm = fmeta[f];
    SNode* nk = nodes + (long long)k * 256;
    Cand* ck = cand + (long long)k * 256 * c.F;
    HistBin* pk = pool + (long long)k * n_hnodes * c.totbins;
    const bool is_used = used[(long long)k * c.F + f] != 0;
    long long ag[4], ah[4];
    const int bslot = ROOT ? 0 : pi;
#pragma unroll
    for (int j = 0; j < 4; ++j) { ag[j] = 0; ah[j] = 0; }
    for (int x = 0; x < lc.gx; ++x) {
        const HistBin* src = part + (((long long)k * lc.gx + x) * lc.max_built + bslot) * c.totbins + fm.hoff;
#pragma unroll
        for (int j = 0; j < 4; ++j) { const int b = lane * 4 + j; if (b < fm.nbins) { const HistBin v = src[b]; ag[j] += v.g; ah[j] += v.h; } }
    }
    if (ROOT) {
        HistBin* h0 = pk + fm.hoff;
        long long sg_ = 0, sh_ = 0;
#pragma unroll
        for (int j = 0; j < 4; ++j) { const int b = lane * 4 + j; if (b < fm.nbins) { HistBin v; v.g = ag[j]; v.h = ah[j]; h0[b] = v; } sg_ += ag[j]; sh_ += ah[j]; }
#pragma unroll
        for (int o = 32; o >= 1; o >>= 1) { sg_ += __shfl_xor(sg_, o); sh_ += __shfl_xor(sh_, o); }
        if (f == 0 && lane == 0) { nk[0].Gq = sg_; nk[0].Hq = sh_; nk[0].searched = 1; atomicAdd(stat_rows, (unsigned long long)pp->n_in); }
        if (!is_used) { if (lane == 0) ck[f].gain = -INFINITY; return; }
        scan_child(ag, ah, fm, sg_, sh_, pp->n_in, c, &ck[f]);
        return;
    }
    const int p = pp->exp[pi];
    const SNode P = nk[p];
    const int l = P.left, r = P.right;
    const bool bl = pp->built_is_left[pi] != 0;
    const int me = side == 0 ? l : r;
    const bool i_am_built = (side == 0) == bl;
    const HistBin* hp = pk + (long long)P.hslot * c.totbins + fm.hoff;
    HistBin* hm = pk + (long long)nk[me].hslot * c.totbins + fm.hoff;
    if (!i_am_built) {
#pragma unroll
        for (int j = 0; j < 4; ++j) {
            const int b = lane * 4 + j;
            if (b < fm.nbins) { const HistBin par = hp[b]; ag[j] = par.g - ag[j]; ah[j] = par.h - ah[j]; } else { ag[j] = 0; ah[j] = 0; }
        }
    }
#pragma unroll
    for (int j = 0; j < 4; ++j) { const int b = lane * 4 + j; if (b < fm.nbins) { HistBin v; v.g = ag[j]; v.h = ah[j]; hm[b] = v; } }
    int nl = count[(long long)k * 256 + l], nr = count[(long long)k * 256 + r];
    {
        const int nb = bl ? nl : nr, ns = P.count - nb;
        if (bl) nr = ns; else nl = ns;
        if (f == 0 && lane == 0 && side == 0) {
            const int sib = bl ? r : l;
            count[(long long)k * 256 + sib] = ns;
            if (lc.sib_local && count_local != count) count_local[(long long)k * 256 + sib] = ns;
        }
    }
    const bool go = !(nr < c.min_data_in_leaf * 2 && nl < c.min_data_in_leaf * 2);
    if (f == 0 && lane == 0) {
        nk[me].count = side == 0 ? nl : nr; nk[me].searched = go ? 1 : 0;
        if (side == 0) atomicAdd(stat_rows, (unsigned long long)(bl ? nl : nr));
    }
    if (!go) return;
    if (!is_used) { if (lane == 0) ck[(long long)me * c.F + f].gain = -INFINITY; return; }
    const long long lGq = P.best.left_gq, lHq = P.best.left_hq;
    if (side == 0) scan_child(ag, ah, fm, lGq, lHq, (long long)nl, c, &ck[(long long)l * c.F + f]);
    else scan_child(ag, ah, fm, P.Gq - lGq, P.Hq - lHq, (long long)nr, c, &ck[(long long)r * c.F + f]);
}

__global__ __launch_bounds__(256) void k_level_plan(LvPlan* __restrict__ plan, SNode* __restrict__ nodes,
                                                    const Cand* __restrict__ cand, const FeatMeta* __restrict__ fmeta,
                                                    int level, TrainConst c, LevelConst lc) {
    __shared__ double pm[256];
    const int k = blockIdx.x, lane = lane_id(), wave = threadIdx.x >> 6;
    LvPlan* pp = &plan[k];
    if (pp->done) return;
    SNode* nk = nodes + (long long)k * 256;
    const Cand* ck = cand + (long long)k * 256 * c.F;
    const int first = pp->lvl_first, end = pp->lvl_end, nlev = end - first;
    for (int n = first + wave; n < end; n += 4) {
        if (!nk[n].searched) { if (lane == 0) { nk[n].best.gain = -INFINITY; nk[n].best_feature = -1; } continue; }
        const Cand* cf = ck + (long long)n * c.F;
        double bg = -INFINITY; int bf = -1;
        for (int f = lane; f < c.F; f += 64) { const double g = cf[f].gain; if (g > -INFINITY && leaf_better(g, f, 0, bg, bf, 0)) { bg = g; bf = f; } }
#pragma unroll
        for (int o = 32; o >= 1; o >>= 1) { const double g2 = __shfl_xor(bg, o); const int f2 = __shfl_xor(bf, o); if (leaf_better(g2, f2, 0, bg, bf, 0)) { bg = g2; bf = f2; } }
        if (lane == 0) {
            if (bf >= 0) { nk[n].best = cf[bf]; nk[n].best_feature = bf; } else { nk[n].best.gain = -INFINITY; nk[n].best_feature = -1; }
        }
    }
    __syncthreads();
    if (wave != 0) return;
    for (int n = lane; n < first; n += 64) pm[n] = nk[n].pmin;
    __syncthreads();
    if (lane < nlev) {
        const int n = first + lane;
        const double g = nk[n].best.gain;
        const int par = nk[n].parent;
        double v = g;
        if (par >= 0) { const double pv = pm[par]; v = (pv < g) ? pv : g; }
        if (!(g > -INFINITY)) v = -INFINITY;
        pm[n] = v; nk[n].pmin = v;
    }
    __syncthreads();
    bool expand = false;
    if (lane < nlev) {
        const double v = pm[first + lane];
        if (v > 0.0) {
            int rank = 0;
            for (int y = 0; y < end; ++y) rank += (pm[y] > v) ? 1 : 0;
            expand = rank < c.num_leaves - 1;
        }
    }
    const unsigned long long em = __ballot(expand);
    const int n_exp = __popcll(em);
    for (int i = lane; i < 256; i += 64) { pp->route0[i] = 0; pp->route1[i] = 0xFFFFFFFFu; }
    __syncthreads();
    if (n_exp == 0) { if (lane == 0) { pp->done = 1; pp->n_exp = 0; pp->n_built = 0; } return; }
    const int child_first = pp->n_nodes;
    const bool with_hist = level < c.max_depth;
    const int hs0 = pp->n_hslots;
    if (expand) {
        const int ei = __popcll(em & ((1ull << lane) - 1ull));
        const int n = first + lane;
        const SNode P = nk[n];
        const int l = child_first + 2 * ei, r = l + 1;
        const int f = P.best_feature;
        const bool built_left = P.best.left_hq * 2 <= P.Hq;
        nk[n].left = l; nk[n].right = r;
        SNode L; memset(&L, 0, sizeof(L));
        L.depth = P.depth + 1; L.parent = n; L.left = -1; L.right = -1; L.best_feature = -1; L.searched = 0; L.best.gain = -INFINITY; L.pmin = -INFINITY;
        SNode R = L;
        L.is_left = 1; L.Gq = P.best.left_gq; L.Hq = P.best.left_hq; L.hslot = with_hist ? hs0 + 2 * ei : -1;
        R.is_left = 0; R.Gq = P.Gq - P.best.left_gq; R.Hq = P.Hq - P.best.left_hq; R.hslot = with_hist ? hs0 + 2 * ei + 1 : -1;
        nk[l] = L; nk[r] = R;
        pp->exp[ei] = (uint8_t)n; pp->built_is_left[ei] = built_left ? 1 : 0;
        const int nanbin = fmeta[f].has_nan ? fmeta[f].V : 255;
        pp->route0[n] = (uint32_t)f | ((uint32_t)(P.best.theta + 1) & 0xFFu) << 8 | (uint32_t)nanbin << 16 | 1u << 24 | (uint32_t)(P.best.dleft ? 1 : 0) << 25;
        const uint32_t ls = with_hist && built_left ? (uint32_t)ei : 0xFFu, rs = with_hist && !built_left ? (uint32_t)ei : 0xFFu;
        pp->route1[n] = (uint32_t)l | (uint32_t)r << 8 | ls << 16 | rs << 24;
    }
    const int n_built = with_hist ? n_exp : 0;
    long long live = expand ? (long long)nk[first + lane].count : 0ll;
#pragma unroll
    for (int o = 32; o >= 1; o >>= 1) live += __shfl_xor(live, o);
    if (lane == 0) {
        pp->live_rows = (int32_t)(live > 0x7FFFFFFFll ? 0x7FFFFFFFll : live);
        pp->n_exp = n_exp; pp->n_built = n_built;
        pp->child_first = child_first; pp->n_nodes = child_first + 2 * n_exp;
        pp->lvl_first = child_first; pp->lvl_end = child_first + 2 * n_exp;
        if (with_hist) pp->n_hslots = hs0 + 2 * n_exp;
    }
}

__global__ __launch_bounds__(64) void k_level_replay(LvPlan* __restrict__ plan, const SNode* __restrict__ nodes, const int32_t* __restrict__ count,
                                                     TreeOut out, const double* __restrict__ init, double* __restrict__ node_delta ,
                                                     int32_t* __restrict__ leaf_node_out ,
                                                     int32_t* __restrict__ any_split, int32_t* __restrict__ err_flag, const int32_t* __restrict__ itp, TrainConst c) {
    const int it = *itp;
    __shared__ int leaf_node[LV_MAX_LEAVES], leaf_parent[LV_MAX_LEAVES], leaf_isleft[LV_MAX_LEAVES];
    __shared__ int node_leaf[256];
    __shared__ double upd[LV_MAX_LEAVES];
    const int k = blockIdx.x, lane = lane_id();
    LvPlan* pp = &plan[k];
    const SNode* nk = nodes + (long long)k * 256;
    const long long tbase = (long long)it * c.K + k;
    const long long nb = tbase * (c.num_leaves - 1);
    double* lv = out.leaf_value + tbase * c.num_leaves;
    const int n_nodes = pp->n_nodes;
    __shared__ double s_gain[256], s_lout[256], s_rout[256], s_lv[LV_MAX_LEAVES];
    __shared__ int s_feat[256], s_theta[256];
    __shared__ short s_left[256], s_right[256], s_parent[256];
    __shared__ unsigned char s_dleft[256];
    for (int n = lane; n < 256; n += 64) {
        node_leaf[n] = -1;
        if (n < n_nodes) {
            const SNode& sn = nk[n];
            const bool se = sn.searched != 0;
            s_gain[n] = se ? sn.best.gain : -INFINITY; s_feat[n] = se ? sn.best_feature : -1;
            s_theta[n] = sn.best.theta; s_dleft[n] = (unsigned char)(sn.best.dleft ? 1 : 0);
            s_lout[n] = sn.best.left_out; s_rout[n] = sn.best.right_out;
            s_left[n] = (short)sn.left; s_right[n] = (short)sn.right; s_parent[n] = (short)sn.parent;
        }
    }
    if (lane == 0) { leaf_node[0] = 0; leaf_parent[0] = -1; leaf_isleft[0] = 0; }
    __syncthreads();
    if (lane == 0) node_leaf[0] = 0;
    __syncthreads();
    int L = 1;
    const int max_leaves = c.num_leaves < LV_MAX_LEAVES ? c.num_leaves : LV_MAX_LEAVES;
    while (L < max_leaves) {
        double bg = -INFINITY; int bf = -1, bl = 0x7FFFFFFF;
        for (int l = lane; l < L; l += 64) {
            const int sn = leaf_node[l];
            const double g = s_gain[sn]; const int f = s_feat[sn];
            if (bl == 0x7FFFFFFF || leaf_better(g, f, l, bg, bf, bl)) { bg = g; bf = f; bl = l; }
        }
#pragma unroll
        for (int o = 32; o >= 1; o >>= 1) {
            const double g2 = __shfl_xor(bg, o); const int f2 = __shfl_xor(bf, o), l2 = __shfl_xor(bl, o);
            if (l2 != 0x7FFFFFFF && (bl == 0x7FFFFFFF || leaf_better(g2, f2, l2, bg, bf, bl))) { bg = g2; bf = f2; bl = l2; }
        }
        if (!(bg > 0.0)) break;
        const int sn = leaf_node[bl];
        const int sl = s_left[sn], sr = s_right[sn];
        if (sl < 0) { if (lane == 0) { pp->error = 1; atomicOr(err_flag, 1); } break; }
        const int node = L - 1, right_leaf = L;
        __syncthreads();
        if (lane == 0) {
            out.feat[nb + node] = bf; out.theta[nb + node] = s_theta[sn]; out.dleft[nb + node] = (int)s_dleft[sn]; out.gain[nb + node] = s_gain[sn];
            out.left[nb + node] = ~bl; out.right[nb + node] = ~right_leaf;
            const int pn = leaf_parent[bl];
            if (pn >= 0) { if (leaf_isleft[bl]) out.left[nb + pn] = node; else out.right[nb + pn] = node; }
            s_lv[bl] = s_lout[sn]; s_lv[right_leaf] = s_rout[sn];
            leaf_node[bl] = sl; leaf_node[right_leaf] = sr;
            leaf_parent[bl] = node; leaf_isleft[bl] = 1; leaf_parent[right_leaf] = node; leaf_isleft[right_leaf] = 0;
            node_leaf[sl] = bl; node_leaf[sr] = right_leaf;
        }
        ++L;
        __syncthreads();
    }
    __syncthreads();
    if (lane == 0) out.L[tbase] = L;
    for (int l = lane; l < L; l += 64) leaf_node_out[(long long)k * LV_MAX_LEAVES + l] = leaf_node[l];
    double* nd = node_delta + (long long)k * 256;
    if (L <= 1) {
        if (lane == 0) lv[0] = (it == 0) ? init[k] : 0.0;
        for (int i = lane; i < 256; i += 64) nd[i] = 0.0;
        return;
    }
    if (lane == 0) atomicOr(any_split + it, 1);
    for (int l = lane; l < L; l += 64) {
        double v = s_lv[l] * c.learning_rate;
        upd[l] = v;
        if (it == 0 && fabs(init[k]) > k_eps()) v += init[k];
        lv[l] = v;
    }
    __syncthreads();
    for (int n = lane; n < 256; n += 64) {
        double d = 0.0;
        if (n < n_nodes) {
            int a = n;
            while (a >= 0 && node_leaf[a] < 0) a = s_parent[a];
            if (a >= 0) d = upd[node_leaf[a]];
        }
        nd[n] = d;
    }
}


__device__ __forceinline__ int lv_final_route(int n, long long row, const uint4* __restrict__ rec, const uint8_t* __restrict__ inbag, const uint32_t* route0,
                                              const uint32_t* route1, int32_t* cnt, int child_first, int lane, const LevelConst& c) {
    const uint32_t w0 = route0[n];
    if (!(w0 & (1u << 24))) return n;
    const int f = (int)(w0 & 0xFFu), theta1 = (int)((w0 >> 8) & 0xFFu), nanbin = (int)((w0 >> 16) & 0xFFu);
    const uint8_t* rec8 = reinterpret_cast<const uint8_t*>(rec);
    const long long last = (long long)(c.nchunk - 1) * c.N + row;
    int bin, mult = 1;
    if (c.has_mult && (f >> 4) == c.nchunk - 1) {
        const uint4 r = rec[last];
        bin = (int)rec_byte(r, f & 15); mult = (int)(r.w >> 24);
    } else {
        bin = (int)rec8[((long long)(f >> 4) * c.N + row) * 16 + (f & 15)];
        if (c.has_mult) mult = (int)rec8[last * 16 + 15];
    }
    const bool left = (bin == nanbin) ? ((w0 >> 25) & 1u) != 0u : (bin < theta1);
    const uint32_t w1 = route1[n];
    n = left ? (int)(w1 & 0xFFu) : (int)((w1 >> 8) & 0xFFu);
    if (!inbag || inbag[row]) atomicAdd(&cnt[(n - child_first) * LV_CNT_REP + (lane & (LV_CNT_REP - 1))], mult);
    return n;
}

template <bool MIS>
__device__ __forceinline__ void lv_final_rows(const uint4* __restrict__ rec, const uint8_t* __restrict__ node, const uint8_t* __restrict__ inbag, double* __restrict__ sk,
                                              const double* nd, const uint32_t* route0, const uint32_t* route1, int32_t* cnt, int child_first, const LevelConst& c) {
    typedef double v2d __attribute__((ext_vector_type(2)));
    const long long N = c.N;
    const int tid = threadIdx.x, lane = tid & 63;
    for (long long i = ((long long)blockIdx.x * 256 + tid) * 4; i < N; i += (long long)gridDim.x * 1024) {
        if (i + 3 < N) {
            const uint32_t n4 = __builtin_nontemporal_load(reinterpret_cast<const uint32_t*>(node + i));
            double sv[4];
            if (MIS) {
                sv[0] = __builtin_nontemporal_load(sk + i);
                const v2d s12 = __builtin_nontemporal_load(reinterpret_cast<const v2d*>(sk + i + 1));
                sv[3] = __builtin_nontemporal_load(sk + i + 3);
                sv[1] = s12.x; sv[2] = s12.y;
            } else {
                const v2d s01 = __builtin_nontemporal_load(reinterpret_cast<const v2d*>(sk + i)), s23 = __builtin_nontemporal_load(reinterpret_cast<const v2d*>(sk + i + 2));
                sv[0] = s01.x; sv[1] = s01.y; sv[2] = s23.x; sv[3] = s23.y;
            }
            if (n4 == 0xFFFFFFFFu) continue;
#pragma unroll
            for (int j = 0; j < 4; ++j) {
                const int n = (int)((n4 >> (8 * j)) & 0xFFu);
                if (n == LV_INACTIVE) continue;
                sv[j] += nd[lv_final_route(n, i + j, rec, inbag, route0, route1, cnt, child_first, lane, c)];
            }
            if (MIS) {
                v2d s12; s12.x = sv[1]; s12.y = sv[2];
                __builtin_nontemporal_store(sv[0], sk + i); __builtin_nontemporal_store(s12, reinterpret_cast<v2d*>(sk + i + 1)); __builtin_nontemporal_store(sv[3], sk + i + 3);
            } else {
                v2d s01, s23; s01.x = sv[0]; s01.y = sv[1]; s23.x = sv[2]; s23.y = sv[3];
                __builtin_nontemporal_store(s01, reinterpret_cast<v2d*>(sk + i)); __builtin_nontemporal_store(s23, reinterpret_cast<v2d*>(sk + i + 2));
            }
            continue;
        }
        for (long long row = i; row < N; ++row) {
            const int n = node[row];
            if (n == LV_INACTIVE) continue;
            sk[row] += nd[lv_final_route(n, row, rec, inbag, route0, route1, cnt, child_first, lane, c)];
        }
    }
}

__global__ __launch_bounds__(256) void k_level_final(const uint4* __restrict__ rec, const uint8_t* __restrict__ node_all,
                                                     const uint8_t* __restrict__ inbag, const LvPlan* __restrict__ plan, const TreeOut out,
                                                     const double* __restrict__ node_delta, double* __restrict__ score, int32_t* __restrict__ count,
                                                     const int32_t* __restrict__ itp, LevelConst c) {
    const int it = *itp;
    __shared__ double nd[256];
    __shared__ uint32_t route0[256], route1[256];
    __shared__ int32_t cnt[2 * LV_MAX_EXP * LV_CNT_REP];
    const int k = blockIdx.y;
    if (out.L[(long long)it * c.K + k] <= 1) return;
    const LvPlan* pp = &plan[k];
    const bool route = !pp->done;
    const int n_exp = route ? pp->n_exp : 0, child_first = pp->child_first;
    const int tid = threadIdx.x;
    nd[tid] = node_delta[(long long)k * 256 + tid];
    route0[tid] = route ? pp->route0[tid] : 0u; route1[tid] = pp->route1[tid];
    for (int i = tid; i < 2 * n_exp * LV_CNT_REP; i += 256) cnt[i] = 0;
    __syncthreads();
    const uint8_t* node = node_all + (long long)k * c.NS;
    double* sk = score + (long long)k * c.N;
    if ((((unsigned long long)sk) & 15ull) == 0ull) lv_final_rows<false>(rec, node, inbag, sk, nd, route0, route1, cnt, child_first, c);
    else lv_final_rows<true>(rec, node, inbag, sk, nd, route0, route1, cnt, child_first, c);
    __syncthreads();
    for (int ci = tid; ci < 2 * n_exp; ci += 256) {
        int tot = 0;
        for (int r2 = 0; r2 < LV_CNT_REP; ++r2) tot += cnt[ci * LV_CNT_REP + r2];
        if (tot) atomicAdd(&count[(long long)k * 256 + child_first + ci], tot);
    }
}

__global__ __launch_bounds__(LV_MAX_LEAVES) void k_level_leafcount(const LvPlan* __restrict__ plan, const int32_t* __restrict__ count,
                                                                   const int32_t* __restrict__ leaf_node, TreeOut out, const int32_t* __restrict__ itp, TrainConst c) {
    const int it = *itp;
    const int k = blockIdx.x, l = threadIdx.x;
    const long long tbase = (long long)it * c.K + k;
    const int L = out.L[tbase];
    if (l >= L) return;
    const int n = leaf_node[(long long)k * LV_MAX_LEAVES + l];
    out.leaf_count[tbase * c.num_leaves + l] = (n == 0) ? (int)plan[k].n_in : count[(long long)k * 256 + n];
}

__global__ void k_next_iteration(int32_t* it) { if (threadIdx.x == 0 && blockIdx.x == 0) it[0] += 1; }

}
```

### spark-data-repair-plugin_amd/csrc/rgbm_small.h

```cpp
#pragma once
#include "rgbm_kernels.h"

namespace rg {

#ifndef SM_THREADS_N
#define SM_THREADS_N 512
#endif
constexpr int SM_THREADS = SM_THREADS_N;
constexpr int SM_WAVES = SM_THREADS / 64;
constexpr int SM_MAX_LEAVES = 256;
constexpr int SM_MAX_FEATS = 255;

struct ScanLane { int32_t feat , bin0 , seg_first , seg_last ; };

__device__ __forceinline__ long long seg_incl_scan(long long v, bool first) {
    const int lane = lane_id();
    int f = first ? 1 : 0;
#pragma unroll
    for (int off = 1; off < 64; off <<= 1) {
        const long long o = __shfl_up(v, off); const int fo = __shfl_up(f, off);
        if (lane >= off && !f) { v += o; f = fo; }
    }
    return v;
}

template <bool REVERSE>
__device__ __forceinline__ ScanBest seg_best_scan(ScanBest v, bool first) {
    const int lane = lane_id();
    int f = first ? 1 : 0;
#pragma unroll
    for (int off = 1; off < 64; off <<= 1) {
        const double g2 = __shfl_up(v.gain, off); const int t2 = __shfl_up(v.theta, off);
        const long long a2 = __shfl_up(v.lg, off), b2 = __shfl_up(v.lh, off); const int fo = __shfl_up(f, off);
        if (lane >= off && !f) {
            if (scan_better<REVERSE>(g2, t2, v.gain, v.theta)) { v.gain = g2; v.theta = t2; v.lg = a2; v.lh = b2; }
            f = fo;
        }
    }
    return v;
}

__device__ void scan_child_packed(const HistBin* hist, const FeatMeta* __restrict__ fmeta, const ScanLane sl, long long Gq, long long Hq, long long num_data,
                                  const TrainConst& c, const uint8_t* __restrict__ used_k, Cand* ck ) {
    const int lane = lane_id();
    const bool on = sl.feat >= 0;
    FeatMeta fm; fm.V = 0; fm.has_nan = 0; fm.nbins = 0; fm.hoff = 0; fm.fast_base = 0; fm.rep_shift = 0; fm.wide_off = 0; fm.pad = 0;
    if (on) fm = fmeta[sl.feat];
    const int V = fm.V;
    const double keps = k_eps();
    const double sum_gradient = (double)Gq * c.inv_sg;
    const double sum_hessian = (double)Hq * c.inv_sh + 2 * keps;
    const double gain_shift = leaf_gain(sum_gradient, sum_hessian, c.l1, c.l2);
    const double min_gain_shift = gain_shift + c.min_gain_to_split;
    const double cnt_factor = (double)num_data / sum_hessian;
    const bool two_way = fm.has_nan && V >= 1;
    long long lg[4], lh[4], lc[4];
    long long tg = 0, th = 0, tc = 0;
#pragma unroll
    for (int j = 0; j < 4; ++j) {
        const int b = sl.bin0 + j;
        const bool val = on && b < V;
        HistBin hb; hb.g = 0; hb.h = 0;
        if (val) hb = hist[fm.hoff + b];
        lg[j] = hb.g; lh[j] = hb.h;
        lc[j] = val ? round_int((double)hb.h * c.inv_sh * cnt_factor) : 0;
        tg += lg[j]; th += lh[j]; tc += lc[j];
    }
    const bool first = !on || sl.seg_first != 0;
    const long long ig = seg_incl_scan(tg, first), ih = seg_incl_scan(th, first), ic = seg_incl_scan(tc, first);
    const int last = on ? sl.seg_last : lane;
    const long long TG = __shfl(ig, last), TH = __shfl(ih, last), TC = __shfl(ic, last);
    long long pg = ig - tg, ph = ih - th, pc = ic - tc;
    ScanBest rv = {-INFINITY, 0, 0, 0}, fw = {-INFINITY, 0, 0, 0};
#pragma unroll
    for (int j = 0; j < 4; ++j) {
        const int b = sl.bin0 + j;
        if (on && b < V) {
            {
                const long long rg = TG - pg, rh = TH - ph, right_count = TC - pc;
                const double sum_right_hessian = (double)rh * c.inv_sh + keps;
                const long long left_count = num_data - right_count;
                const long long lhq = Hq - rh, lgq = Gq - rg;
                const double sum_left_hessian = (double)lhq * c.inv_sh + keps;
                const bool ok = !(right_count < c.min_data_in_leaf || sum_right_hessian < c.min_sum_hessian) &&
                                !(left_count < c.min_data_in_leaf) && !(sum_left_hessian < c.min_sum_hessian);
                if (ok) {
                    const double cur = leaf_gain((double)lgq * c.inv_sg, sum_left_hessian, c.l1, c.l2) +
                                       leaf_gain((double)rg * c.inv_sg, sum_right_hessian, c.l1, c.l2);
                    if (cur > min_gain_shift && scan_better<true>(cur, b - 1, rv.gain, rv.theta)) { rv.gain = cur; rv.theta = b - 1; rv.lg = lgq; rv.lh = lhq; }
                }
            }
            pg += lg[j]; ph += lh[j]; pc += lc[j];
            if (two_way) {
                const long long lgq = pg, lhq = ph, left_count = pc;
                const double sum_left_hessian = (double)lhq * c.inv_sh + keps;
                const long long right_count = num_data - left_count;
                const long long rh = Hq - lhq, rg = Gq - lgq;
                const double sum_right_hessian = (double)rh * c.inv_sh + keps;
                const bool ok = !(left_count < c.min_data_in_leaf || sum_left_hessian < c.min_sum_hessian) &&
                                !(right_count < c.min_data_in_leaf) && !(sum_right_hessian < c.min_sum_hessian);
                if (ok) {
                    const double cur = leaf_gain((double)lgq * c.inv_sg, sum_left_hessian, c.l1, c.l2) +
                                       leaf_gain((double)rg * c.inv_sg, sum_right_hessian, c.l1, c.l2);
                    if (cur > min_gain_shift && scan_better<false>(cur, b, fw.gain, fw.theta)) { fw.gain = cur; fw.theta = b; fw.lg = lgq; fw.lh = lhq; }
                }
            }
        }
    }
    rv = seg_best_scan<true>(rv, first);
    fw = seg_best_scan<false>(fw, first);
    if (on && lane == sl.seg_last) {
        Cand o; o.gain = -INFINITY; o.theta = 0; o.dleft = 1; o.left_gq = 0; o.left_hq = 0; o.left_out = 0.0; o.right_out = 0.0;
        if (used_k[sl.feat]) {
            if (rv.gain > -INFINITY && rv.gain > o.gain + min_gain_shift) {
                o.theta = rv.theta; o.dleft = 1; o.left_gq = rv.lg; o.left_hq = rv.lh;
                const double lH = (double)rv.lh * c.inv_sh + keps, rH = (double)(Hq - rv.lh) * c.inv_sh + keps;
                o.left_out = leaf_output((double)rv.lg * c.inv_sg, lH, c.l1, c.l2);
                o.right_out = leaf_output((double)(Gq - rv.lg) * c.inv_sg, rH, c.l1, c.l2);
                o.gain = rv.gain - min_gain_shift;
            }
            if (fw.gain > -INFINITY && fw.gain > o.gain + min_gain_shift) {
                o.theta = fw.theta; o.dleft = 0; o.left_gq = fw.lg; o.left_hq = fw.lh;
                const double lH = (double)fw.lh * c.inv_sh + keps, rH = (double)(Hq - fw.lh) * c.inv_sh + keps;
                o.left_out = leaf_output((double)fw.lg * c.inv_sg, lH, c.l1, c.l2);
                o.right_out = leaf_output((double)(Gq - fw.lg) * c.inv_sg, rH, c.l1, c.l2);
                o.gain = fw.gain - min_gain_shift;
            }
        }
        ck[sl.feat] = o;
    }
}

struct SmallFit {
    TrainConst c;
    const uint4* rec;
    const int32_t* ycol;
    float2* gh;
    double* score;
    int32_t* idx0; int32_t* idx1;
    int32_t* base_idx;
    HistBin* pool;
    const FeatMeta* fmeta; const ChunkMeta* cmeta;
    const uint8_t* used;
    TreeOut out;
    const double* init; double* upd ; int32_t* tree_L ; int32_t* any_split ;
    const double* class_w; const double* y_value;
    unsigned int* rand_state; const int32_t* sorted_rows; uint8_t* inbag; unsigned int* bagcnt ; int32_t* oob;
    double bag_fraction; long long bag_nrb;
    int32_t bag_freq, tree0 , n_estimators, pad;
    unsigned long long lds_hist;
    const uint4* vrec;
    double* vscore;
    long long n_valid;
    const ScanLane* scan_map;
    int32_t scan_waves, pad2;
    unsigned long long* prof;
};

__host__ __device__ inline size_t sm_hist_area(size_t lds_hist, int num_leaves) {
    const size_t a = lds_hist > (size_t)num_leaves * 8 ? lds_hist : (size_t)num_leaves * 8;
    return (a + 15) & ~(size_t)15;
}
__host__ __device__ inline size_t sm_lds_bytes(size_t lds_hist, int num_leaves, int F, int packed_totbins = 0) {
    size_t b = sm_hist_area(lds_hist, num_leaves);
    b += (size_t)num_leaves * sizeof(Leaf);
    b = (b + 15) & ~(size_t)15;
// ... 359 lines not shown
```

Before: 1.840 million.

## Fuse level split search into one block per node pair with LDS histograms

Replaces the per-feature k_level_split kernel with k_level_step, which runs one block per expanded node pair. That block reduces the partial histograms into LDS, derives the sibling by subtraction, scans all features using the packed scan-lane map, and picks the best candidate in-kernel. This removes the global candidate buffer and the per-node argmax pass in k_level_plan, and skips the separate reduce kernel for non-root levels when gx is small. It also folds the iteration increment into k_level_init and rewrites leaf selection in k_level_replay to keep leaf state in registers with wave shuffles instead of LDS and barriers. In exchange, parallelism per node is lower (a single block) and LDS usage per block is larger.

```diff
diff --git a/spark-data-repair-plugin_amd/csrc/rgbm.hip b/spark-data-repair-plugin_amd/csrc/rgbm.hip
--- a/spark-data-repair-plugin_amd/csrc/rgbm.hip
+++ b/spark-data-repair-plugin_amd/csrc/rgbm.hip
@@ -157,6 +157,9 @@
     int mt_rot = -1;
     int mt_rot_copies2 = 16;
     int mt_rot_tmin = 2;
+    bool step_readback = false;
+    int step_threads = 0;
+    int step_max_gx = 0;
     bool fx_separate = false;
     bool distinct = true;
     double distinct_max_ratio = DISTINCT_MAX_RATIO;
@@ -173,6 +176,9 @@
     if (const char* e = getenv("RGBM_JOINT_ROOT")) w.joint_root = atoi(e) != 0;
     if (const char* e = getenv("RGBM_MT_ACC2")) w.mt_acc2 = atoi(e) != 0;
     if (const char* e = getenv("RGBM_MT_SPARSE")) w.mt_sparse = atoi(e) != 0;
+    if (const char* e = getenv("RGBM_STEP_READBACK")) w.step_readback = atoi(e) != 0;
+    if (const char* e = getenv("RGBM_STEP_THREADS")) w.step_threads = atoi(e);
+    if (const char* e = getenv("RGBM_STEP_MAX_GX")) w.step_max_gx = atoi(e);
     if (const char* e = getenv("RGBM_FX_MEASURE")) w.fx_separate = strcmp(e, "separate") == 0;
     if (const char* e = getenv("RGBM_MT_ROT")) w.mt_rot = atoi(e);
     if (const char* e = getenv("RGBM_MT_ROT_COPIES2")) w.mt_rot_copies2 = atoi(e);
@@ -798,7 +804,9 @@
     bool use_reduce = false;
     bool joint_root = false; int vtotbins = 0;
     DevBuf<rg::FeatMeta> vfmeta; DevBuf<rg::ChunkMeta> vcmeta; DevBuf<uint4> rec_j; DevBuf<rg::HistBin> part_j, red_j; DevBuf<rg::JointFeat> jf; DevBuf<int16_t> binfeat;
-    DevBuf<uint8_t> node; DevBuf<rg::LvPlan> plan; DevBuf<rg::SNode> snodes; DevBuf<rg::Cand> lcand;
+    DevBuf<uint8_t> node; DevBuf<rg::LvPlan> plan; DevBuf<rg::SNode> snodes;
+    DevBuf<rg::ScanLane> scan_map; std::vector<rg::ScanLane> h_scan; int scan_waves = 0; bool step_hist_lds = true;
+    int step_threads = 512, step_max_gx = 256;
     DevBuf<rg::HistBin> part, lpool, part_red; DevBuf<int32_t> count, count_g, err, leafnode; DevBuf<double> ndelta; DevBuf<unsigned long long> d_statrows;
     const int score_gx = (int)std::max<long long>(1, std::min<long long>((st.N + 1023) / 1024, (2048 + st.K - 1) / st.K));
     LevelTrace trace;
@@ -823,9 +831,14 @@
         lc.gx = passes.root_gx; lc.xcd_blocks = 1; lc.max_built = 1;
         node.alloc((size_t)st.K * lc.NS);
         HIPCHK(hipMemsetAsync(node.p, 0xFF, (size_t)st.K * lc.NS, s));
-        plan.alloc(st.K); snodes.alloc((size_t)st.K * 256); lcand.alloc((size_t)st.K * 256 * st.F);
+        plan.alloc(st.K); snodes.alloc((size_t)st.K * 256);
         part.alloc(passes.part_items * st.h.tc.totbins); lpool.alloc((size_t)st.K * n_hnodes * st.h.tc.totbins);
-        count.alloc((size_t)st.K * 256); use_reduce = st.dp || lc.gx > 4;
+        scan_waves = scan_lane_map(st.h.fmeta.data(), st.F, h_scan);
+        scan_map.alloc(h_scan.size()); scan_map.upload(h_scan.data(), h_scan.size(), s);
+        step_hist_lds = ls_hist_in_lds(st.h.tc.totbins, st.F) && !st.sw.step_readback;
+        if (st.sw.step_threads >= 128 && st.sw.step_threads <= LS_MAX_THREADS && st.sw.step_threads % 64 == 0) step_threads = st.sw.step_threads;
+        if (st.sw.step_max_gx >= 1) step_max_gx = st.sw.step_max_gx;
+        count.alloc((size_t)st.K * 256); use_reduce = st.dp || lc.gx > step_max_gx;
         if (st.dp) count_g.alloc((size_t)st.K * 256);
         const int max_built_all = 1 << std::max(0, st.p.max_depth - 2);
         part_red.alloc((size_t)st.K * max_built_all * st.h.tc.totbins + (size_t)st.K * 128 );
@@ -885,7 +898,7 @@
     }
     std::pair<const rg::HistBin*, rg::LevelConst> exchange(bool root, int nb, const rg::LevelConst& lp) {
         using namespace rg;
-        if (root && !use_reduce) return {part.p, lp};
+        if (root ? !use_reduce : (!st.dp && lp.gx <= step_max_gx)) return {part.p, lp};
         if (root && joint_root) {
             hipLaunchKernelGGL(k_level_reduce, dim3((vtotbins + 63) / 64, 1, st.K), dim3(256), 0, s, part_j.p, red_j.p, plan.p, count.p, 1, 1, lcj);
             hipLaunchKernelGGL(k_level_marginal, dim3((st.h.tc.totbins + 255) / 256, st.K), dim3(256), 0, s, red_j.p, part_red.p, plan.p, count.p, jf.p, binfeat.p, vtotbins, lc);
@@ -904,7 +917,8 @@
         const TreeOut to = st.trees.out();
         trace.cur_it = it;
         trace.sum("gh", st.gh.p, (size_t)st.K * st.h.tc.NG * 8);
-        hipLaunchKernelGGL(k_level_init, dim3(st.K), dim3(64), 0, s, plan.p, snodes.p, count.p, st.n_in_ptr, (long long)st.h.n_train, st.fxq.p, st.h.tc.fx, st.fxs.p, lc);
+        hipLaunchKernelGGL(k_level_init, dim3(st.K), dim3(64), 0, s, plan.p, snodes.p, count.p, st.n_in_ptr, (long long)st.h.n_train, st.fxq.p, st.h.tc.fx, st.fxs.p, st.it.p, lc);
+        const size_t step_lds = ls_lds_bytes(st.h.tc.totbins, st.F, step_hist_lds);
         int32_t* cntg = st.dp ? count_g.p : count.p;
         st.timers.timed(true, [&]() {
             if (joint_root)
@@ -916,12 +930,12 @@
         });
         {
             auto ex = exchange(true, 1, lc);
-            hipLaunchKernelGGL(k_level_split<true>, dim3((st.F + 3) / 4, 1, st.K), dim3(256), 0, s, ex.first, lpool.p, plan.p, snodes.p, cntg, count.p, st.bins.fmeta.p,
-                               st.used.p, lcand.p, d_statrows.p, st.it.p, n_hnodes, st.fxs.p, st.h.tc, ex.second);
+            hipLaunchKernelGGL(k_level_step<true>, dim3(1, st.K), dim3(step_threads), step_lds, s, ex.first, lpool.p, plan.p, snodes.p, cntg, count.p, st.bins.fmeta.p,
+                               st.used.p, scan_map.p, scan_waves, step_hist_lds ? 1 : 0, d_statrows.p, st.it.p, n_hnodes, st.fxs.p, st.h.tc, ex.second);
             trace_level(0);
         }
         for (int level = 1; level < st.p.max_depth; ++level) {
-            hipLaunchKernelGGL(k_level_plan, dim3(st.K), dim3(256), 0, s, plan.p, snodes.p, lcand.p, st.bins.fmeta.p, level, st.h.tc, lc);
+            hipLaunchKernelGGL(k_level_plan, dim3(st.K), dim3(64), 0, s, plan.p, snodes.p, st.bins.fmeta.p, level, st.h.tc, lc);
             LevelConst lp = lc;
             lp.xcd_blocks = 0; lp.gx = passes.mt_gx[level]; lp.max_built = 1 << (level - 1);
             for (const MtLaunch& L : passes.mt[level]) {
@@ -936,18 +950,17 @@
                 });
             }
             auto ex = exchange(false, 1 << (level - 1), lp);
-            hipLaunchKernelGGL(k_level_split<false>, dim3((st.F + 1) / 2, 1 << (level - 1), st.K), dim3(256), 0, s, ex.first, lpool.p, plan.p, snodes.p,
-                               cntg, count.p, st.bins.fmeta.p, st.used.p, lcand.p, d_statrows.p, st.it.p, n_hnodes, st.fxs.p, st.h.tc, ex.second);
+            hipLaunchKernelGGL(k_level_step<false>, dim3(1 << (level - 1), st.K), dim3(step_threads), step_lds, s, ex.first, lpool.p, plan.p, snodes.p,
+                               cntg, count.p, st.bins.fmeta.p, st.used.p, scan_map.p, scan_waves, step_hist_lds ? 1 : 0, d_statrows.p, st.it.p, n_hnodes, st.fxs.p, st.h.tc, ex.second);
             trace_level(level);
         }
-        hipLaunchKernelGGL(k_level_plan, dim3(st.K), dim3(256), 0, s, plan.p, snodes.p, lcand.p, st.bins.fmeta.p, st.p.max_depth, st.h.tc, lc);
+        hipLaunchKernelGGL(k_level_plan, dim3(st.K), dim3(64), 0, s, plan.p, snodes.p, st.bins.fmeta.p, st.p.max_depth, st.h.tc, lc);
         hipLaunchKernelGGL(k_level_replay, dim3(st.K), dim3(64), 0, s, plan.p, snodes.p, cntg, to, st.init.p, ndelta.p, leafnode.p, st.trees.any.p, err.p, st.it.p, st.h.tc);
         hipLaunchKernelGGL(k_level_final, dim3(score_gx, st.K), dim3(256), 0, s, st.bins.rec.p, node.p, st.bag.inbag.p, plan.p, to, ndelta.p, st.score.p, count.p, st.it.p, lc);
         if (st.dp) { hipLaunchKernelGGL(k_copy_i32, dim3(st.K), dim3(256), 0, s, count.p, count_g.p, (long long)st.K * 256); all_reduce(count_g.p, (size_t)st.K * 256, AR_I32, s); }
         hipLaunchKernelGGL(k_level_leafcount, dim3(st.K), dim3(LV_MAX_LEAVES), 0, s, plan.p, cntg, leafnode.p, to, st.it.p, st.h.tc);
         trace_level(st.p.max_depth);
         trace.sum("score", st.score.p, (size_t)st.K * st.N * 8); trace.sum("node", node.p, (size_t)st.K * lc.NS);
-        hipLaunchKernelGGL(k_next_iteration, dim3(1), dim3(1), 0, s, st.it.p);
     }
     void enqueue_report() { err.download(&h_err, 1, s); d_statrows.download(&statrows, 1, s); }
     void report(int32_t target_col) {
@@ -1103,7 +1116,7 @@
         HIPCHK(hipStreamSynchronize(s));
         st.n_in_ptr = st.dp ? st.bagcnt_g.p : st.bag.bagcnt.p;
     }
-    st.it.alloc(1); st.it.zero(s);
+    st.it.alloc(1); HIPCHK(hipMemsetAsync(st.it.p, 0xFF, sizeof(int32_t), s));
     st.alloc_fx_parts();
     unsigned int view_train_rows = 0;
     if (view_stats && stats) {
@@ -1246,15 +1259,8 @@
         try {
         fit_setup(tab, sp.y_value, sp.class_weight, nullptr, p, F, h);
         {
-            std::vector<ScanLane> sm; int lanes_used = 0;
-            for (int f = 0; f < F; ++f) {
-                const int nl_f = std::max(1, (h.fmeta[f].V + 3) / 4);
-                if (lanes_used % 64 + nl_f > 64) while (lanes_used % 64) { sm.push_back(ScanLane{-1, 0, 1, 0}); ++lanes_used; }
-                const int first = lanes_used % 64;
-                for (int q = 0; q < nl_f; ++q) { sm.push_back(ScanLane{f, 4 * q, q == 0 ? 1 : 0, first + nl_f - 1}); ++lanes_used; }
-            }
-            while (lanes_used % 64) { sm.push_back(ScanLane{-1, 0, 1, 0}); ++lanes_used; }
-            const int Wn = lanes_used / 64;
+            std::vector<ScanLane> sm;
+            const int Wn = scan_lane_map(h.fmeta.data(), F, sm);
             const bool off_switch = getenv("RGBM_SMALL_PACKED") && atoi(getenv("RGBM_SMALL_PACKED")) == 0;
             if (!off_switch && 2 * Wn <= SM_WAVES && h.tc.totbins <= 2048 && sm_lds_bytes(h.lds_hist, NL, F, h.tc.totbins) <= 150 * 1024) { d.scan_waves = Wn; d.h_scan = std::move(sm); }
         }
diff --git a/spark-data-repair-plugin_amd/csrc/rgbm_level.h b/spark-data-repair-plugin_amd/csrc/rgbm_level.h
--- a/spark-data-repair-plugin_amd/csrc/rgbm_level.h
+++ b/spark-data-repair-plugin_amd/csrc/rgbm_level.h
@@ -1,5 +1,6 @@
 #pragma once
 #include "rgbm_kernels.h"
+#include "rgbm_small.h"
 
 namespace rg {
 
@@ -163,8 +164,10 @@
 
 __global__ __launch_bounds__(64) void k_level_init(LvPlan* __restrict__ plan, SNode* __restrict__ nodes, int32_t* __restrict__ count,
                                                    const unsigned int* __restrict__ n_in_ptr, long long n_train,
-                                                   unsigned long long* __restrict__ Q, FxGrid fx, FxScale* __restrict__ fxs, LevelConst c) {
+                                                   unsigned long long* __restrict__ Q, FxGrid fx, FxScale* __restrict__ fxs,
+                                                   int32_t* __restrict__ itp , LevelConst c) {
     const int k = blockIdx.x, lane = lane_id();
+    if (k == 0 && lane == 0) itp[0] += 1;
     if (lane == 0) {
         const int e_g = fx_tree_exponent(Q[2 * k], fx.q_mult, fx.c_g, fx.e_g_min, fx.e_g_max);
         const int e_h = fx_tree_exponent(Q[2 * k + 1], fx.q_mult, fx.c_h, fx.e_h_min, fx.e_h_max);
@@ -935,112 +938,138 @@
     count_g[i] = (int32_t)cnt64[i];
 }
 
+constexpr int LS_MAX_THREADS = 1024;
+constexpr int LS_LDS_BUDGET = 64 * 1024;
+__host__ __device__ inline size_t ls_lds_bytes(int totbins, int F, bool hist_lds) { return (hist_lds ? (size_t)2 * totbins * sizeof(HistBin) : 0) + (size_t)2 * F * sizeof(Cand); }
+inline bool ls_hist_in_lds(int totbins, int F) { return ls_lds_bytes(totbins, F, true) + 1024 <= (size_t)LS_LDS_BUDGET; }
+
 template <bool ROOT>
-__global__ __launch_bounds__(256) void k_level_split(const HistBin* __restrict__ part, HistBin* __restrict__ pool, LvPlan* __restrict__ plan,
-                                                     SNode* __restrict__ nodes, int32_t* __restrict__ count, int32_t* __restrict__ count_local,
-                                                     const FeatMeta* __restrict__ fmeta, const uint8_t* __restrict__ used_all ,
-                                                     Cand* __restrict__ cand , unsigned long long* __restrict__ stat_rows,
-                                                     const int32_t* __restrict__ itp ,
-                                                     int n_hnodes, const FxScale* __restrict__ fxs, TrainConst c_model, LevelConst lc) {
-    const int k = blockIdx.z, pi = blockIdx.y;
-    const TrainConst c = tree_const(c_model, fxs, k);
-    const uint8_t* used = used_all + (long long)(*itp) * c.K * c.F;
-    const int wv = threadIdx.x >> 6;
-    const int f = ROOT ? blockIdx.x * 4 + wv : blockIdx.x * 2 + (wv >> 1);
-    const int side = wv & 1;
+__global__ __launch_bounds__(LS_MAX_THREADS) void k_level_step(const HistBin* __restrict__ part, HistBin* __restrict__ pool, const LvPlan* __restrict__ plan,
+                                                               SNode* __restrict__ nodes, int32_t* __restrict__ count, int32_t* __restrict__ count_local,
+                                                               const FeatMeta* __restrict__ fmeta, const uint8_t* __restrict__ used_all ,
+                                                               const ScanLane* __restrict__ scan_map , int scan_waves, int hist_lds,
+                                                               unsigned long long* __restrict__ stat_rows, const int32_t* __restrict__ itp ,
+                                                               int n_hnodes, const FxScale* __restrict__ fxs, TrainConst c_model, LevelConst lc) {
+    extern __shared__ __attribute__((aligned(16))) unsigned char smem[];
+    const int k = blockIdx.y, pi = blockIdx.x;
     const LvPlan* pp = &plan[k];
     if (pp->done) return;
     if (!ROOT && pi >= pp->n_exp) return;
-    if (f >= c.F) return;
-    const int lane = lane_id();
-    const FeatMeta fm = fmeta[f];
+    const int T = blockDim.x, tid = threadIdx.x, lane = tid & 63, wv = tid >> 6, nwaves = T >> 6;
+    const int tb = lc.totbins, F = lc.F;
+    const int l = ROOT ? 0 : pp->child_first + 2 * pi, r = ROOT ? 0 : l + 1;
+    const bool bl = ROOT ? true : pp->built_is_left[pi] != 0;
+    const long long n_in = pp->n_in;
     SNode* nk = nodes + (long long)k * 256;
-    Cand* ck = cand + (long long)k * 256 * c.F;
-    HistBin* pk = pool + (long long)k * n_hnodes * c.totbins;
-    const bool is_used = used[(long long)k * c.F + f] != 0;
-    long long ag[4], ah[4];
-    const int bslot = ROOT ? 0 : pi;
-#pragma unroll
-    for (int j = 0; j < 4; ++j) { ag[j] = 0; ah[j] = 0; }
-    for (int x = 0; x < lc.gx; ++x) {
-        const HistBin* src = part + (((long long)k * lc.gx + x) * lc.max_built + bslot) * c.totbins + fm.hoff;
-#pragma unroll
-        for (int j = 0; j < 4; ++j) { const int b = lane * 4 + j; if (b < fm.nbins) { const HistBin v = src[b]; ag[j] += v.g; ah[j] += v.h; } }
+    int nl = ROOT ? 0 : count[(long long)k * 256 + l], nr = ROOT ? 0 : count[(long long)k * 256 + r];
+    const int hs_l = ROOT ? 0 : nk[l].hslot, hs_r = ROOT ? 0 : nk[r].hslot;
+    const int p = ROOT ? 0 : (int)pp->exp[pi];
+    long long P_Gq = 0, P_Hq = 0, P_lGq = 0, P_lHq = 0; int P_count = 0, P_hslot = 0;
+    if (!ROOT) { const SNode& P = nk[p]; P_Gq = P.Gq; P_Hq = P.Hq; P_lGq = P.best.left_gq; P_lHq = P.best.left_hq; P_count = P.count; P_hslot = P.hslot; }
+    const TrainConst c = tree_const(c_model, fxs, k);
+    const uint8_t* used_k = used_all + ((long long)(*itp) * lc.K + k) * F;
+    HistBin* pk = pool + (long long)k * n_hnodes * tb;
+    HistBin* gL = pk + (long long)hs_l * tb; HistBin* gR = pk + (long long)hs_r * tb;
+    HistBin* hL = hist_lds ? reinterpret_cast<HistBin*>(smem) : gL;
+    HistBin* hR = hist_lds ? reinterpret_cast<HistBin*>(smem) + tb : gR;
+    Cand* ck = reinterpret_cast<Cand*>(smem + (hist_lds ? (size_t)2 * tb * sizeof(HistBin) : 0));
+    HistBin* hbuilt = bl ? hL : hR; HistBin* hsib = bl ? hR : hL;
+
+    {
+        const int bslot = ROOT ? 0 : pi;
+        const HistBin* src = part + (((long long)k * lc.gx) * lc.max_built + bslot) * tb;
+        const long long xs = (long long)lc.max_built * tb;
+        const int nbl = tb >= T ? T : ((tb + 63) & ~63);
+        int PL = hist_lds ? T / nbl : 1;
+        if (PL > lc.gx) PL = lc.gx;
+        if (PL > 1) {
+            for (int b = tid; b < tb; b += T) { HistBin z; z.g = 0; z.h = 0; hbuilt[b] = z; }
+            __syncthreads();
+            const int b = tid % nbl, xl = tid / nbl;
+            if (b < tb && xl < PL) {
+                long long ag = 0, ah = 0;
+#pragma unroll 8
+                for (int x = xl; x < lc.gx; x += PL) { const HistBin v = src[x * xs + b]; ag += v.g; ah += v.h; }
+                atomicAdd(reinterpret_cast<unsigned long long*>(&hbuilt[b].g), (unsigned long long)ag);
+                atomicAdd(reinterpret_cast<unsigned long long*>(&hbuilt[b].h), (unsigned long long)ah);
+            }
+        } else {
+            for (int b = tid; b < tb; b += T) {
+                long long ag = 0, ah = 0;
+#pragma unroll 8
+                for (int x = 0; x < lc.gx; ++x) { const HistBin v = src[x * xs + b]; ag += v.g; ah += v.h; }
+                HistBin o; o.g = ag; o.h = ah; hbuilt[b] = o;
+            }
+        }
+        __syncthreads();
     }
     if (ROOT) {
-        HistBin* h0 = pk + fm.hoff;
-        long long sg_ = 0, sh_ = 0;
-#pragma unroll
-        for (int j = 0; j < 4; ++j) { const int b = lane * 4 + j; if (b < fm.nbins) { HistBin v; v.g = ag[j]; v.h = ah[j]; h0[b] = v; } sg_ += ag[j]; sh_ += ah[j]; }
-#pragma unroll
-        for (int o = 32; o >= 1; o >>= 1) { sg_ += __shfl_xor(sg_, o); sh_ += __shfl_xor(sh_, o); }
-        if (f == 0 && lane == 0) { nk[0].Gq = sg_; nk[0].Hq = sh_; nk[0].searched = 1; atomicAdd(stat_rows, (unsigned long long)pp->n_in); }
-        if (!is_used) { if (lane == 0) ck[f].gain = -INFINITY; return; }
-        scan_child(ag, ah, fm, sg_, sh_, pp->n_in, c, &ck[f]);
-        return;
-    }
-    const int p = pp->exp[pi];
-    const SNode P = nk[p];
-    const int l = P.left, r = P.right;
-    const bool bl = pp->built_is_left[pi] != 0;
-    const int me = side == 0 ? l : r;
-    const bool i_am_built = (side == 0) == bl;
-    const HistBin* hp = pk + (long long)P.hslot * c.totbins + fm.hoff;
-    HistBin* hm = pk + (long long)nk[me].hslot * c.totbins + fm.hoff;
-    if (!i_am_built) {
-#pragma unroll
-        for (int j = 0; j < 4; ++j) {
-            const int b = lane * 4 + j;
-            if (b < fm.nbins) { const HistBin par = hp[b]; ag[j] = par.g - ag[j]; ah[j] = par.h - ah[j]; } else { ag[j] = 0; ah[j] = 0; }
-        }
-    }
-#pragma unroll
-    for (int j = 0; j < 4; ++j) { const int b = lane * 4 + j; if (b < fm.nbins) { HistBin v; v.g = ag[j]; v.h = ah[j]; hm[b] = v; } }
-    int nl = count[(long long)k * 256 + l], nr = count[(long long)k * 256 + r];
-    {
-        const int nb = bl ? nl : nr, ns = P.count - nb;
+        if (hist_lds) for (int b = tid; b < tb; b += T) gL[b] = hL[b];
+    } else {
+        const HistBin* hp = pk + (long long)P_hslot * tb;
+        HistBin* gbuilt = bl ? gL : gR; HistBin* gsib = bl ? gR : gL;
+        for (int b = tid; b < tb; b += T) {
+            const HistBin bu = hbuilt[b], par = hp[b];
+            HistBin sb; sb.g = par.g - bu.g; sb.h = par.h - bu.h;
+            hsib[b] = sb;
+            if (hist_lds) { gbuilt[b] = bu; gsib[b] = sb; }
+        }
+    }
+    bool go = true;
+    if (!ROOT) {
+        const int nb = bl ? nl : nr, ns = P_count - nb;
         if (bl) nr = ns; else nl = ns;
-        if (f == 0 && lane == 0 && side == 0) {
+        go = !(nr < c.min_data_in_leaf * 2 && nl < c.min_data_in_leaf * 2);
+        if (tid == 0) {
             const int sib = bl ? r : l;
             count[(long long)k * 256 + sib] = ns;
             if (lc.sib_local && count_local != count) count_local[(long long)k * 256 + sib] = ns;
-        }
-    }
-    const bool go = !(nr < c.min_data_in_leaf * 2 && nl < c.min_data_in_leaf * 2);
-    if (f == 0 && lane == 0) {
-        nk[me].count = side == 0 ? nl : nr; nk[me].searched = go ? 1 : 0;
-        if (side == 0) atomicAdd(stat_rows, (unsigned long long)(bl ? nl : nr));
-    }
-    if (!go) return;
-    if (!is_used) { if (lane == 0) ck[(long long)me * c.F + f].gain = -INFINITY; return; }
-    const long long lGq = P.best.left_gq, lHq = P.best.left_hq;
-    if (side == 0) scan_child(ag, ah, fm, lGq, lHq, (long long)nl, c, &ck[(long long)l * c.F + f]);
-    else scan_child(ag, ah, fm, P.Gq - lGq, P.Hq - lHq, (long long)nr, c, &ck[(long long)r * c.F + f]);
-}
-
-__global__ __launch_bounds__(256) void k_level_plan(LvPlan* __restrict__ plan, SNode* __restrict__ nodes,
-                                                    const Cand* __restrict__ cand, const FeatMeta* __restrict__ fmeta,
-                                                    int level, TrainConst c, LevelConst lc) {
+            nk[l].count = nl; nk[l].searched = go ? 1 : 0;
+            nk[r].count = nr; nk[r].searched = go ? 1 : 0;
+            atomicAdd(stat_rows, (unsigned long long)nb);
+        }
+    }
+    __syncthreads();
+    const int nch = ROOT ? 1 : 2;
+    if (go) {
+        for (int ws = wv; ws < nch * scan_waves; ws += nwaves) {
+            const int child = ws / scan_waves, slot = ws - child * scan_waves;
+            const ScanLane sl = scan_map[slot * 64 + lane];
+            if (ROOT) {
+                const FeatMeta f0 = fmeta[0];
+                long long sg_ = 0, sh_ = 0;
+#pragma unroll
+                for (int j = 0; j < 4; ++j) { const int b = lane * 4 + j; if (b < f0.nbins) { const HistBin v = hL[f0.hoff + b]; sg_ += v.g; sh_ += v.h; } }
+#pragma unroll
+                for (int o = 32; o >= 1; o >>= 1) { sg_ += __shfl_xor(sg_, o); sh_ += __shfl_xor(sh_, o); }
+                if (ws == 0 && lane == 0) { nk[0].Gq = sg_; nk[0].Hq = sh_; nk[0].searched = 1; atomicAdd(stat_rows, (unsigned long long)n_in); }
+                scan_child_packed(hL, fmeta, sl, sg_, sh_, n_in, c, used_k, ck);
+            } else if (child == 0) scan_child_packed(hL, fmeta, sl, P_lGq, P_lHq, (long long)nl, c, used_k, ck);
+            else scan_child_packed(hR, fmeta, sl, P_Gq - P_lGq, P_Hq - P_lHq, (long long)nr, c, used_k, ck + F);
+        }
+    }
+    __syncthreads();
+    if (wv < nch) {
+        const int n = ROOT ? 0 : (wv == 0 ? l : r);
+        const Cand* cf = ck + wv * F;
+        double bg = -INFINITY; int bf = -1;
+        if (go) for (int f = lane; f < F; f += 64) { const double g = cf[f].gain; if (g > -INFINITY && leaf_better(g, f, 0, bg, bf, 0)) { bg = g; bf = f; } }
+#pragma unroll
+        for (int o = 32; o >= 1; o >>= 1) { const double g2 = __shfl_xor(bg, o); const int f2 = __shfl_xor(bf, o); if (leaf_better(g2, f2, 0, bg, bf, 0)) { bg = g2; bf = f2; } }
+        if (lane == 0) {
+            if (bf >= 0) { nk[n].best = cf[bf]; nk[n].best_feature = bf; } else { nk[n].best.gain = -INFINITY; nk[n].best_feature = -1; }
+        }
+    }
+}
+
+__global__ __launch_bounds__(64) void k_level_plan(LvPlan* __restrict__ plan, SNode* __restrict__ nodes, const FeatMeta* __restrict__ fmeta,
+                                                   int level, TrainConst c, LevelConst lc) {
     __shared__ double pm[256];
-    const int k = blockIdx.x, lane = lane_id(), wave = threadIdx.x >> 6;
+    const int k = blockIdx.x, lane = lane_id();
     LvPlan* pp = &plan[k];
     if (pp->done) return;
     SNode* nk = nodes + (long long)k * 256;
-    const Cand* ck = cand + (long long)k * 256 * c.F;
     const int first = pp->lvl_first, end = pp->lvl_end, nlev = end - first;
-    for (int n = first + wave; n < end; n += 4) {
-        if (!nk[n].searched) { if (lane == 0) { nk[n].best.gain = -INFINITY; nk[n].best_feature = -1; } continue; }
-        const Cand* cf = ck + (long long)n * c.F;
-        double bg = -INFINITY; int bf = -1;
-        for (int f = lane; f < c.F; f += 64) { const double g = cf[f].gain; if (g > -INFINITY && leaf_better(g, f, 0, bg, bf, 0)) { bg = g; bf = f; } }
-#pragma unroll
-        for (int o = 32; o >= 1; o >>= 1) { const double g2 = __shfl_xor(bg, o); const int f2 = __shfl_xor(bf, o); if (leaf_better(g2, f2, 0, bg, bf, 0)) { bg = g2; bf = f2; } }
-        if (lane == 0) {
-            if (bf >= 0) { nk[n].best = cf[bf]; nk[n].best_feature = bf; } else { nk[n].best.gain = -INFINITY; nk[n].best_feature = -1; }
-        }
-    }
-    __syncthreads();
-    if (wave != 0) return;
     for (int n = lane; n < first; n += 64) pm[n] = nk[n].pmin;
     __syncthreads();
     if (lane < nlev) {
@@ -1108,7 +1137,7 @@
                                                      int32_t* __restrict__ leaf_node_out ,
                                                      int32_t* __restrict__ any_split, int32_t* __restrict__ err_flag, const int32_t* __restrict__ itp, TrainConst c) {
     const int it = *itp;
-    __shared__ int leaf_node[LV_MAX_LEAVES], leaf_parent[LV_MAX_LEAVES], leaf_isleft[LV_MAX_LEAVES];
+    __shared__ int leaf_parent[LV_MAX_LEAVES], leaf_isleft[LV_MAX_LEAVES];
     __shared__ int node_leaf[256];
     __shared__ double upd[LV_MAX_LEAVES];
     const int k = blockIdx.x, lane = lane_id();
@@ -1133,46 +1162,60 @@
             s_left[n] = (short)sn.left; s_right[n] = (short)sn.right; s_parent[n] = (short)sn.parent;
         }
     }
-    if (lane == 0) { leaf_node[0] = 0; leaf_parent[0] = -1; leaf_isleft[0] = 0; }
+    if (lane == 0) { leaf_parent[0] = -1; leaf_isleft[0] = 0; }
     __syncthreads();
     if (lane == 0) node_leaf[0] = 0;
     __syncthreads();
+    static_assert(LV_MAX_LEAVES <= 128, "two leaves per lane");
+    double lg[2] = {-INFINITY, -INFINITY}; int lf[2] = {-1, -1}, ln[2] = {0, 0};
+    if (lane == 0) { lg[0] = s_gain[0]; lf[0] = s_feat[0]; }
     int L = 1;
     const int max_leaves = c.num_leaves < LV_MAX_LEAVES ? c.num_leaves : LV_MAX_LEAVES;
     while (L < max_leaves) {
-        double bg = -INFINITY; int bf = -1, bl = 0x7FFFFFFF;
-        for (int l = lane; l < L; l += 64) {
-            const int sn = leaf_node[l];
-            const double g = s_gain[sn]; const int f = s_feat[sn];
-            if (bl == 0x7FFFFFFF || leaf_better(g, f, l, bg, bf, bl)) { bg = g; bf = f; bl = l; }
-        }
-#pragma unroll
-        for (int o = 32; o >= 1; o >>= 1) {
-            const double g2 = __shfl_xor(bg, o); const int f2 = __shfl_xor(bf, o), l2 = __shfl_xor(bl, o);
-            if (l2 != 0x7FFFFFFF && (bl == 0x7FFFFFFF || leaf_better(g2, f2, l2, bg, bf, bl))) { bg = g2; bf = f2; bl = l2; }
-        }
-        if (!(bg > 0.0)) break;
-        const int sn = leaf_node[bl];
+        const bool up = leaf_better(lg[1], lf[1], lane + 64, lg[0], lf[0], lane);
+        const double g = up ? lg[1] : lg[0]; const int f = up ? lf[1] : lf[0], l = up ? lane + 64 : lane, n = up ? ln[1] : ln[0];
+        double m = g;
+#pragma unroll
+        for (int o = 32; o >= 1; o >>= 1) { const double m2 = __shfl_xor(m, o); m = m2 > m ? m2 : m; }
+        if (!(m > 0.0)) break;
+        unsigned long long tie = __ballot(g == m);
+        int wl = __ffsll((long long)tie) - 1;
+        if (tie & (tie - 1ull)) {
+            const int fk = (g == m) ? (f < 0 ? 0x7FFFFFFF : f) : 0x7FFFFFFF;
+            int fmin = fk;
+#pragma unroll
+            for (int o = 32; o >= 1; o >>= 1) { const int f2 = __shfl_xor(fmin, o); fmin = f2 < fmin ? f2 : fmin; }
+            int lmin = (g == m && fk == fmin) ? l : 0x7FFFFFFF;
+#pragma unroll
+            for (int o = 32; o >= 1; o >>= 1) { const int l2 = __shfl_xor(lmin, o); lmin = l2 < lmin ? l2 : lmin; }
+            wl = lmin & 63;
+        }
+        const int wpk = __shfl(n | (l >> 6) << 8, wl);
+        const int sn = wpk & 0xFF, bl = wl + 64 * (wpk >> 8), bf = s_feat[sn];
         const int sl = s_left[sn], sr = s_right[sn];
         if (sl < 0) { if (lane == 0) { pp->error = 1; atomicOr(err_flag, 1); } break; }
         const int node = L - 1, right_leaf = L;
-        __syncthreads();
         if (lane == 0) {
             out.feat[nb + node] = bf; out.theta[nb + node] = s_theta[sn]; out.dleft[nb + node] = (int)s_dleft[sn]; out.gain[nb + node] = s_gain[sn];
             out.left[nb + node] = ~bl; out.right[nb + node] = ~right_leaf;
             const int pn = leaf_parent[bl];
             if (pn >= 0) { if (leaf_isleft[bl]) out.left[nb + pn] = node; else out.right[nb + pn] = node; }
             s_lv[bl] = s_lout[sn]; s_lv[right_leaf] = s_rout[sn];
-            leaf_node[bl] = sl; leaf_node[right_leaf] = sr;
             leaf_parent[bl] = node; leaf_isleft[bl] = 1; leaf_parent[right_leaf] = node; leaf_isleft[right_leaf] = 0;
             node_leaf[sl] = bl; node_leaf[sr] = right_leaf;
         }
+        const double gl_ = s_gain[sl], gr_ = s_gain[sr]; const int fl_ = s_feat[sl], fr_ = s_feat[sr];
+#pragma unroll
+        for (int s2 = 0; s2 < 2; ++s2) {
+            if (lane + 64 * s2 == bl) { lg[s2] = gl_; lf[s2] = fl_; ln[s2] = sl; }
+            if (lane + 64 * s2 == right_leaf) { lg[s2] = gr_; lf[s2] = fr_; ln[s2] = sr; }
+        }
         ++L;
-        __syncthreads();
     }
     __syncthreads();
     if (lane == 0) out.L[tbase] = L;
-    for (int l = lane; l < L; l += 64) leaf_node_out[(long long)k * LV_MAX_LEAVES + l] = leaf_node[l];
+    if (lane < L) leaf_node_out[(long long)k * LV_MAX_LEAVES + lane] = ln[0];
+    if (lane + 64 < L) leaf_node_out[(long long)k * LV_MAX_LEAVES + lane + 64] = ln[1];
     double* nd = node_delta + (long long)k * 256;
     if (L <= 1) {
         if (lane == 0) lv[0] = (it == 0) ? init[k] : 0.0;
@@ -1305,6 +1348,4 @@
     out.leaf_count[tbase * c.num_leaves + l] = (n == 0) ? (int)plan[k].n_in : count[(long long)k * 256 + n];
 }
 
-__global__ void k_next_iteration(int32_t* it) { if (threadIdx.x == 0 && blockIdx.x == 0) it[0] += 1; }
-
-}
+}
diff --git a/spark-data-repair-plugin_amd/csrc/rgbm_small.h b/spark-data-repair-plugin_amd/csrc/rgbm_small.h
--- a/spark-data-repair-plugin_amd/csrc/rgbm_small.h
+++ b/spark-data-repair-plugin_amd/csrc/rgbm_small.h
@@ -1,4 +1,6 @@
 #pragma once
+#include <algorithm>
+#include <vector>
 #include "rgbm_kernels.h"
 
 namespace rg {
@@ -12,6 +14,19 @@
 constexpr int SM_MAX_FEATS = 255;
 
 struct ScanLane { int32_t feat , bin0 , seg_first , seg_last ; };
+
+inline int scan_lane_map(const FeatMeta* fm, int F, std::vector<ScanLane>& sm) {
+    sm.clear();
+    int lanes_used = 0;
+    for (int f = 0; f < F; ++f) {
+        const int nl_f = std::max(1, (fm[f].V + 3) / 4);
+        if (lanes_used % 64 + nl_f > 64) while (lanes_used % 64) { sm.push_back(ScanLane{-1, 0, 1, 0}); ++lanes_used; }
+        const int first = lanes_used % 64;
+        for (int q = 0; q < nl_f; ++q) { sm.push_back(ScanLane{f, 4 * q, q == 0 ? 1 : 0, first + nl_f - 1}); ++lanes_used; }
+    }
+    while (lanes_used % 64) { sm.push_back(ScanLane{-1, 0, 1, 0}); ++lanes_used; }
+    return lanes_used / 64;
+}
 
 __device__ __forceinline__ long long seg_incl_scan(long long v, bool first) {
     const int lane = lane_id();
```

New measurement: 1.891 million, median of 6. 1.03x the previous value.
